# lambdaclass/mina_bridge

Hardware: AMD Instinct MI355X
Metric: Mina state proofs verified/sec (batch) (higher is better)
Workload: dtype u32x8-montgomery (255-bit prime fields, integer)

## Files before the change

include/mina_verify.h:

```cpp
#ifndef MINA_VERIFY_H
#define MINA_VERIFY_H

#include <stddef.h>
#include <stdint.h>

#ifdef __cplusplus
extern "C" {
#endif

#define MINA_OK 0
#define MINA_ERR_ARG (-1)
#define MINA_ERR_HIP (-2)
#define MINA_ERR_STATE (-3)
#define MINA_ERR_FORMAT (-4)

#define MINA_FIELD_FP 0
#define MINA_FIELD_FQ 1
#define MINA_CURVE_PALLAS 0
#define MINA_CURVE_VESTA 1

typedef struct mina_ctx mina_ctx;

int mina_ctx_create(int device_id, mina_ctx **out);
void mina_ctx_destroy(mina_ctx *ctx);
// ... 67 lines not shown

int mina_to_group(mina_ctx *ctx, int curve, size_t n, const uint8_t *t, uint8_t *out_affine);

int mina_field_mul(mina_ctx *ctx, int field, size_t n, const uint8_t *a, const uint8_t *b, uint8_t *out);
int mina_field_inv(mina_ctx *ctx, int field, size_t n, const uint8_t *a, uint8_t *out);
int mina_field_sqrt(mina_ctx *ctx, int field, size_t n, const uint8_t *a, uint8_t *out, uint8_t *out_is_square);
int mina_selftest_group_law(mina_ctx *ctx, int curve, size_t n, const uint8_t *p_affine, const uint8_t *q_affine,
                            uint8_t *out_serial, uint8_t *out_quad, uint8_t *same);
#define MINA_FE29_IN_OPERANDS 8
#define MINA_FE29_OUT_RESULTS 4
#define MINA_FE29_FLAG_NEG 1
#define MINA_FE29_FLAG_OK 1
#define MINA_FE29_FLAG_INF 2
#define MINA_FE29_MUL_ASM 0
#define MINA_FE29_SQR_ASM 1
#define MINA_FE29_DOT2_ASM 2
#define MINA_FE29_DOT3_ASM 3
#define MINA_FE29_SQR_HI_ASM 4
#define MINA_FE29_MUL_HI_ASM 5
#define MINA_FE29_MUL_LZ 6
#define MINA_FE29_SQR_LZ 7
#define MINA_FE29_MUL_HI_LZ 8
#define MINA_FE29_MULRC_LZ 9
#define MINA_FE29_DOT2RC_LZ 10
#define MINA_FE29_DOT3RC_LZ 11
#define MINA_FE29_MUL_SG 12
#define MINA_FE29_SQR_SG 13
#define MINA_FE29_MUL_HI_SG 14
#define MINA_FE29_SQR_HI_SG 15
#define MINA_FE29_MULRC_SG 16
#define MINA_FE29_DOT2RC_SG 17
#define MINA_FE29_DOT3RC_SG 18
#define MINA_FE29_ROW1_SG 19
#define MINA_FE29_SUB_KP_ONE 32
#define MINA_FE29_KP_MINUS_NEG_Y 33
#define MINA_FE29_KP_MINUS_SUB_X1 34
#define MINA_FE29_KP_MINUS_SUB_Y1 35
#define MINA_FE29_KP_MINUS_G_U1 36
#define MINA_FE29_KP_MINUS_G_S1 37
#define MINA_FE29_KP_MINUS_A_2B_X3_SUB 38
#define MINA_FE29_KP_MINUS_A_2B_G_X3_SUB 39
#define MINA_FE29_ADD_KP_MINUS_SUB_X3 40
#define MINA_FE29_ADD_KP_MINUS_G_SUB_X3 41
#define MINA_FE29_ADD 42
#define MINA_FE29_ADD3 43
#define MINA_FE29_WORDS 44
#define MINA_FE29_IS_MULTIPLE_OF_P 45
#define MINA_FE29_LEAVE 46
#define MINA_FE29_ADD_AFFINE 64
#define MINA_FE29_ADD_AFFINE_TWIN 65
#define MINA_FE29_XYZZ_ADD 66
#define MINA_FE29_XYZZ_LEAVE 67
int mina_selftest_fe29(mina_ctx *ctx, int field, int op, size_t n, const uint32_t *rows_in , uint32_t *rows_out );
#define MINA_FE32_IN_OPERANDS 8
#define MINA_FE32_OUT_RESULTS 4
#define MINA_FE32_FLAG_TRUE 1
#define MINA_FE32_FLAG_LANES_AGREE 2
#define MINA_FE32_COND_SUB_P 0
#define MINA_FE32_ADD 1
#define MINA_FE32_SUB 2
#define MINA_FE32_NEG 3
#define MINA_FE32_DBL 4
#define MINA_FE32_MUL 5
#define MINA_FE32_SQR 6
#define MINA_FE32_DOT2 7
#define MINA_FE32_DOT3 8
// ... 350 lines not shown
```

mina_bridge_amd/csrc/api_account.hip:

```cpp
#include <mutex>

#include "ctx.h"
#include <chrono>
#include <new>
#include "sponge.cuh"
#include "wire_account.h"

int mb_merkle_fold_dev(mina_ctx *c, int field, size_t n, uint32_t depth, const uint32_t *d_leaves, const uint32_t *d_sib, const uint8_t *d_dirs, uint32_t *d_roots);
int mb_merkle_prepare_salts(mina_ctx *c, int field, uint32_t depth);
int mb_ensure_state_salts(mina_ctx *c);

namespace mb {

template <int F, int LANES>
__global__ void __launch_bounds__(256)
salted_hash_kernel(uint32_t n, FieldK fk, const PoseidonParams *__restrict__ pp, const fe_t *__restrict__ salts, const uint32_t *__restrict__ salt_idx,
                   const uint32_t *__restrict__ records , const uint32_t *__restrict__ nfields,
                   const uint32_t *__restrict__ patch_a, uint32_t slot_a, const uint32_t *__restrict__ patch_b, uint32_t slot_b, uint32_t *__restrict__ out ) {
    __builtin_amdgcn_s_setprio(3);
    bool writer;
    const uint32_t sp = coop_sponge_index<LANES>(writer), e = coop_elem<LANES>();
    const bool live = sp < n;
    const uint32_t idx = live ? sp : 0;
    const uint32_t *rec = records + (size_t)idx * MINA_PSTATE_SLOTS * 8;
    uint32_t nf = nfields[idx]; if (nf > MINA_PSTATE_SLOTS) nf = MINA_PSTATE_SLOTS;
    fe_t s = salts[salt_idx[idx] * 3 + e];
    uint32_t count = 0;
    for (uint32_t el = 0; el < nf; ++el) {
        if (count == 2) { poseidon_permute_coop<F, LANES>(s, pp); count = 0; }
        if (e == count) {
            const uint32_t *src = (patch_a && el == slot_a) ? patch_a + (size_t)idx * 8 : ((patch_b && el == slot_b) ? patch_b + (size_t)idx * 8 : rec + (size_t)el * 8);
            s = fe_add<F>(s, fe_to_mont<F>(load_fe<F>(src), fk.r2));
        }
        ++count;
    }
    poseidon_permute_coop<F, LANES>(s, pp);
    s = coop_get<LANES>(s, 0);
    if (live && writer) { const fe_t w = fe_from_mont<F>(s); for (int i = 0; i < 8; ++i) out[(size_t)sp * 8 + i] = w.v[i]; }
}

}

static int salted_hash_dev(mina_ctx *c, size_t n, const uint32_t *salt_idx, const uint32_t *recs, const uint32_t *nf, const uint32_t *pa, uint32_t sa,
                           const uint32_t *pb, uint32_t sb, uint32_t *out) {
    const PoseidonParams *pp = c->pparams[FIELD_FP].as<PoseidonParams>();
    const fe_t *salts = c->state_salts.as<fe_t>();
    ProfScope ps_(c, PS_STATE_HASH);
    return with_lanes<16, 8, 3>(hash_lanes(c, n, n), [&](auto lanes) {
        constexpr int LN = decltype(lanes)::value;
        mb::salted_hash_kernel<FIELD_FP, LN><<<cdiv(coop_threads<LN>(n), 256), 256, 0, c->L->stream>>>((uint32_t)n, c->fk[FIELD_FP], pp, salts, salt_idx, recs, nf, pa, sa, pb, sb, out);
        HIPC(hipGetLastError());
        return MINA_OK;
    });
}

namespace {
struct ParsedAccount { bool ok = false, abi_ok = false; mw::Account acc; uint32_t depth = 0; uint8_t sib[64 * 32]; uint8_t dirs[64]; uint8_t ledger[32]; };

void parse_account(const uint8_t *proof, size_t proof_len, const uint8_t *pub, size_t pub_len, ParsedAccount &pa) {
    if (!proof || !pub) return;
    size_t acc_off = 0, eo = 0, el = 0;
    if (mina_parse_merkle_path(proof, proof_len, 64, pa.sib, pa.dirs, &pa.depth, &acc_off) != MINA_OK) return;
    if (mina_parse_account_pub_inputs(pub, pub_len, pa.ledger, &eo, &el) != MINA_OK) return;
    mw::Bincode c(proof + acc_off, proof_len - acc_off);
    if (!mw::read_account(c, pa.acc) || c.pos != proof_len - acc_off) return;
    pa.ok = true;
    std::vector<uint8_t> enc;
    mw::abi_encode_account(pa.acc, enc);
    pa.abi_ok = enc.size() == el && memcmp(enc.data(), pub + eo, el) == 0;
}

}

static int account_hashes(mina_ctx *c, const std::vector<const mw::Account *> &accs, uint8_t *hashes_out, uint32_t depth, const uint8_t *sib, const uint8_t *dirs, uint8_t *roots_out,
                          Lane *lane = nullptr, std::mutex *enq_mu = nullptr) {
    const size_t n = accs.size();
    if (n == 0) return MINA_OK;
    int rc;
    struct Enq {
        mina_ctx *c; Lane *lane; std::mutex *mu; bool held = false;
        void lock() { if (mu) mu->lock(); held = true; if (lane) c->L = lane; else c->use_lane0(); }
// ... 127 lines not shown
```

mina_bridge_amd/csrc/api_account_dev.hip:

```cpp
#include <mutex>

#include "ctx.h"
#include "account_pack.cuh"
#include "wire_account.h"

int mb_merkle_prepare_salts(mina_ctx *c, int field, uint32_t depth);
int mb_ensure_state_salts(mina_ctx *c);

static_assert(mb::ACCT_SALT_URI == MB_SALT_ZKAPP_URI && mb::ACCT_SALT_VK == MB_SALT_SIDE_LOADED_VK && mb::ACCT_SALT_ZKAPP == MB_SALT_ZKAPP_ACCOUNT && mb::ACCT_SALT_ACCOUNT == MB_SALT_ACCOUNT &&
              mb::ACCT_SALT_VK == MB_N_PREFIX_SALTS - 1, "account_pack.cuh names the salts of ctx.h");
static_assert(mb::ZR_URI_HASH == mw::ZK_SLOT_URI && mb::ZR_VK_HASH == mw::ZK_SLOT_VK, "the zkApp record's patched slots (wire_account.h)");

static constexpr size_t ACCOUNT_MAX_PROOFS = (size_t)1 << 22;
static constexpr size_t REC_BYTES = (size_t)MINA_PSTATE_SLOTS * 32;

static int acct_hash_dev(mina_ctx *c, size_t n, uint32_t roles, const uint32_t *count_dev, const uint32_t *salt_idx, const uint32_t *recs, const uint32_t *nf, const uint32_t *pa, uint32_t sa,
                         const uint32_t *pb, uint32_t sb, const uint32_t *marks, const uint32_t *pa_default, const uint32_t *out_index, uint32_t *out) {
    const PoseidonParams *pp = c->pparams[FIELD_FP].as<PoseidonParams>();
    const fe_t *salts = c->state_salts.as<fe_t>();
    ProfScope ps_(c, PS_STATE_HASH);
    return with_lanes<16, 8, 3>(hash_lanes(c, n, n * roles), [&](auto lanes) {
        constexpr int LN = decltype(lanes)::value;
        mb::acct_hash_kernel<FIELD_FP, LN><<<cdiv(coop_threads<LN>(n * roles), 256), 256, 0, c->L->stream>>>((uint32_t)n, roles, count_dev, c->fk[FIELD_FP], pp, salts, salt_idx, recs, nf, pa, sa,
                                                                                                           pb, sb, marks, pa_default, out_index, out);
        HIPC(hipGetLastError());
        return MINA_OK;
    });
}

static constexpr size_t DEF_RECS = 96, DEF_NF = DEF_RECS + 3 * REC_BYTES, DEF_SALT = DEF_NF + 12, DEF_BYTES = DEF_SALT + 12;
static int ensure_defaults(mina_ctx *c) {
    if (c->have_acct_defaults) return MINA_OK;
    int rc;
    if ((rc = c->acct_defaults.ensure(DEF_BYTES))) return rc;
    std::vector<uint8_t> host(DEF_BYTES, 0);
    uint32_t *nf = (uint32_t *)(host.data() + DEF_NF), *salt = (uint32_t *)(host.data() + DEF_SALT);
    const mw::ZkappAccount z;
    std::vector<mw::B32> f;
    auto put = [&](size_t k, uint32_t salt_id) { for (size_t j = 0; j < f.size() && j < MINA_PSTATE_SLOTS; ++j) memcpy(host.data() + DEF_RECS + k * REC_BYTES + j * 32, f[j].b, 32);
                                                 nf[k] = (uint32_t)(f.size() < MINA_PSTATE_SLOTS ? f.size() : MINA_PSTATE_SLOTS); salt[k] = salt_id; };
    mw::zkapp_uri_fields(z.zkapp_uri, f); put(0, MB_SALT_ZKAPP_URI);
    mw::vk_fields(mw::dummy_vk(), f); put(1, MB_SALT_SIDE_LOADED_VK);
    mw::zkapp_fields(z, f); put(2, MB_SALT_ZKAPP_ACCOUNT);
    uint8_t *d = c->acct_defaults.as<uint8_t>();
    uint32_t *h = c->acct_defaults.as<uint32_t>();
    HIPC(hipMemcpyAsync(d, host.data(), DEF_BYTES, hipMemcpyHostToDevice, c->L->stream));
    const uint32_t *recs = (const uint32_t *)(d + DEF_RECS), *dnf = (const uint32_t *)(d + DEF_NF), *dsalt = (const uint32_t *)(d + DEF_SALT);
    if ((rc = acct_hash_dev(c, 1, 2, nullptr, dsalt, recs, dnf, nullptr, 0, nullptr, 0, nullptr, nullptr, nullptr, h))) return rc;
    if ((rc = acct_hash_dev(c, 1, 1, nullptr, dsalt + 2, recs + 2 * REC_BYTES / 4, dnf + 2, h, mw::ZK_SLOT_URI, h + 8, mw::ZK_SLOT_VK, nullptr, nullptr, nullptr, h + 16))) return rc;
    HIPC(hipStreamSynchronize(c->L->stream));
    c->have_acct_defaults = true;
    return MINA_OK;
}

// ... 18 lines not shown
    }
};

static int frontend_launch(mina_ctx *c, size_t n, const void *d_blob, size_t blob_len, const void *d_proof_off, const void *d_proof_len, const void *d_pub_off, const void *d_pub_len,
                           void *d_records, void *d_nfields, void *d_salt_idx, void *d_siblings, void *d_dirs, void *d_depths, void *d_ledger, void *d_marks, void *d_zk_index,
                           void *d_zk_count, void *d_bits) {
    HIPC(hipMemsetAsync(d_zk_count, 0, 4, c->L->stream));
    mb::acct_frontend_kernel<<<cdiv(n, 256), 256, 0, c->L->stream>>>((uint32_t)n, (const uint8_t *)d_blob, (uint64_t)blob_len, (const uint64_t *)d_proof_off, (const uint64_t *)d_proof_len,
                                                                   (const uint64_t *)d_pub_off, (const uint64_t *)d_pub_len, (uint4 *)d_records, (uint32_t *)d_nfields, (uint32_t *)d_salt_idx,
                                                                   (uint4 *)d_siblings, (uint8_t *)d_dirs, (uint32_t *)d_depths, (uint4 *)d_ledger, (uint32_t *)d_marks, (uint32_t *)d_zk_index,
                                                                   (uint32_t *)d_zk_count, (uint32_t *)d_bits);
    HIPC(hipGetLastError());
    return MINA_OK;
}

static int account_job_on_lane(mina_ctx *c, size_t n, const void *d_blob, size_t blob_len, const void *d_proof_off, const void *d_proof_len, const void *d_pub_off, const void *d_pub_len,
                               void *d_passed, void *d_ran, void *d_account_hashes, void *d_roots) {
    Lane &L = *c->L;
    const AccountWs w(n);
    int rc;
    if ((rc = L.ac_ws.ensure(w.total))) return rc;
    uint8_t *d = L.ac_ws.as<uint8_t>();
    auto W = [&](size_t off) { return (uint32_t *)(d + off); };
    auto stage = [&](size_t off, uint32_t s, size_t per) { return (const uint32_t *)(d + off + (size_t)s * n * per); };
    if ((rc = frontend_launch(c, n, d_blob, blob_len, d_proof_off, d_proof_len, d_pub_off, d_pub_len, d + w.records, d + w.nfields, d + w.salt_idx, d + w.siblings, d + w.dirs, d + w.depths,
                              d + w.ledger, d + w.marks, d + w.zk_index, d + w.zk_count, d + w.bits))) return rc;
    const uint32_t *defaults = c->acct_defaults.as<uint32_t>(), *zk_count = W(w.zk_count);
    if ((rc = acct_hash_dev(c, n, 2, zk_count, stage(w.salt_idx, mb::AS_URI, 4), stage(w.records, mb::AS_URI, REC_BYTES), stage(w.nfields, mb::AS_URI, 4), nullptr, 0, nullptr, 0, nullptr, nullptr,
                            nullptr, W(w.h_uri)))) return rc;
    if ((rc = acct_hash_dev(c, n, 1, zk_count, stage(w.salt_idx, mb::AS_ZKAPP, 4), stage(w.records, mb::AS_ZKAPP, REC_BYTES), stage(w.nfields, mb::AS_ZKAPP, 4), W(w.h_uri), mw::ZK_SLOT_URI,
                            W(w.h_uri) + n * 8, mw::ZK_SLOT_VK, nullptr, nullptr, W(w.zk_index), W(w.h_zkapp)))) return rc;
    if ((rc = acct_hash_dev(c, n, 1, nullptr, stage(w.salt_idx, mb::AS_ACCOUNT, 4), stage(w.records, mb::AS_ACCOUNT, REC_BYTES), stage(w.nfields, mb::AS_ACCOUNT, 4), W(w.h_zkapp), mb::AR_ZKAPP_HASH,
                            nullptr, 0, W(w.marks), defaults + 16, nullptr, W(w.h_account)))) return rc;
    if ((rc = with_lanes<16, 8, 3>(merkle_lanes(c, n), [&](auto lanes) {
            constexpr int LN = decltype(lanes)::value;
            mb::acct_fold_kernel<FIELD_FP, LN><<<cdiv(coop_threads<LN>(n), 256), 256, 0, L.stream>>>((uint32_t)n, c->fk[FIELD_FP], c->pparams[FIELD_FP].as<PoseidonParams>(),
                c->merkle_salts[FIELD_FP].as<fe_t>(), W(w.h_account), W(w.siblings), d + w.dirs, W(w.depths), W(w.roots));
            HIPC(hipGetLastError());
            return MINA_OK;
        }))) return rc;
    mb::acct_verdict_kernel<<<cdiv(n, 256), 256, 0, L.stream>>>((uint32_t)n, W(w.bits), (const uint4 *)(d + w.roots), (const uint4 *)(d + w.ledger), (uint32_t *)d_passed, (uint32_t *)d_ran);
    HIPC(hipGetLastError());
    if (d_account_hashes) HIPC(hipMemcpyAsync(d_account_hashes, d + w.h_account, n * 32, hipMemcpyDeviceToDevice, L.stream));
    if (d_roots) HIPC(hipMemcpyAsync(d_roots, d + w.roots, n * 32, hipMemcpyDeviceToDevice, L.stream));
    return MINA_OK;
}

static bool misaligned8(const void *a, const void *b, const void *c2, const void *d) { return (((uintptr_t)a | (uintptr_t)b | (uintptr_t)c2 | (uintptr_t)d) & 7u) != 0; }

extern "C" int mina_account_frontend_dev(mina_ctx *c, size_t n, const void *d_blob, size_t blob_len, const void *d_proof_off, const void *d_proof_len, const void *d_pub_off,
                                         const void *d_pub_len, void *d_records, void *d_nfields, void *d_salt_idx, void *d_siblings, void *d_dirs, void *d_depths, void *d_ledger_hashes,
                                         void *d_zk_marks, void *d_zk_index, void *d_zk_count, void *d_bits) {
    if (!c || !d_zk_count || (n && (!d_blob || !d_proof_off || !d_proof_len || !d_pub_off || !d_pub_len || !d_records || !d_nfields || !d_salt_idx || !d_siblings || !d_dirs || !d_depths ||
                                    !d_ledger_hashes || !d_zk_marks || !d_zk_index || !d_bits))) return fail(MINA_ERR_ARG, "null argument");
    if (misaligned8(d_proof_off, d_proof_len, d_pub_off, d_pub_len) || (((uintptr_t)d_records | (uintptr_t)d_siblings | (uintptr_t)d_ledger_hashes) & 15u) ||
        (((uintptr_t)d_nfields | (uintptr_t)d_salt_idx | (uintptr_t)d_depths | (uintptr_t)d_zk_marks | (uintptr_t)d_zk_index | (uintptr_t)d_zk_count | (uintptr_t)d_bits) & 3u))
        return fail(MINA_ERR_ARG, "misaligned argument: offsets / lengths 8, records / siblings / ledger hashes 16, the u32 arrays 4 bytes");
    if (n > ACCOUNT_MAX_PROOFS) return fail(MINA_ERR_ARG, "n too large");
    if (!c->have_pparams[FIELD_FP]) return fail(MINA_ERR_STATE, "Poseidon constants not installed for Fp");
    HIPC(hipSetDevice(c->device));
    c->next_lane();
    if (n == 0) { HIPC(hipMemsetAsync(d_zk_count, 0, 4, c->L->stream)); return MINA_OK; }
    return frontend_launch(c, n, d_blob, blob_len, d_proof_off, d_proof_len, d_pub_off, d_pub_len, d_records, d_nfields, d_salt_idx, d_siblings, d_dirs, d_depths, d_ledger_hashes, d_zk_marks,
                           d_zk_index, d_zk_count, d_bits);
}

extern "C" int mina_account_job_dev(mina_ctx *c, size_t n, const void *d_blob, size_t blob_len, const void *d_proof_off, const void *d_proof_len, const void *d_pub_off, const void *d_pub_len,
// ... 59 lines not shown
```

mina_bridge_amd/csrc/api_core.hip:

```cpp
#include "ctx.h"
#include "sponge.cuh"
#include "msm.cuh"

#include <sys/random.h>
#include <atomic>
#include <condition_variable>
#include <deque>
#include <mutex>

template <int F> static fe_t host_modulus() { fe_t p; for (int i = 0; i < 8; ++i) p.v[i] = modulus_limb<F>(i); return p; }
static void fe_shr1(fe_t &a) { for (int i = 0; i < 7; ++i) a.v[i] = (a.v[i] >> 1) | (a.v[i + 1] << 31); a.v[7] >>= 1; }
static fe_t fe_sub_small(const fe_t &a, uint32_t k) { fe_t r = a; uint64_t br = k; for (int i = 0; i < 8 && br; ++i) { uint64_t t = (uint64_t)r.v[i] - br; r.v[i] = (uint32_t)t; br = (t >> 32) & 1u; } return r; }
static fe_t fe_div3(const fe_t &a) { fe_t r; uint64_t rem = 0; for (int i = 7; i >= 0; --i) { uint64_t cur = (rem << 32) | a.v[i]; r.v[i] = (uint32_t)(cur / 3); rem = cur % 3; } return r; }

template <int F> static FieldK make_field_consts() {
    FieldK k;
    fe_t p = host_modulus<F>();
    fe_t a = fe_zero(); a.v[0] = 1;
    for (int i = 0; i < 512; ++i) { a = fe_add<F>(a, a); if (i == 255) k.one = a; }
    k.r2 = a;
    fe_t pm1 = fe_sub_small(p, 1);
    k.pm2 = fe_sub_small(p, 2);
    k.pm1d2 = pm1; fe_shr1(k.pm1d2);
    k.half = k.pm1d2;
// ... 24 lines not shown
    if (ndev <= 0) return fail(MINA_ERR_HIP, "no HIP device: libminaverify has no CPU fallback");
    if (device_id < 0 || device_id >= ndev) return fail(MINA_ERR_ARG, "bad device id");
    HIPC(hipSetDevice(device_id));
    mina_ctx *c = new mina_ctx();
    c->device = device_id;
    hipError_t e = hipStreamCreateWithFlags(&c->lanes[0].stream, hipStreamNonBlocking);
    if (e != hipSuccess) { delete c; return fail(MINA_ERR_HIP, "hipStreamCreate failed"); }
    c->use_lane0();
    c->fk[FIELD_FP] = make_field_consts<FIELD_FP>();
    c->fk[FIELD_FQ] = make_field_consts<FIELD_FQ>();
    c->state_frontend = mb_state_frontend_on_lane;
    c->account_on_device = mb_verify_account_dev_on;
    *out = c;
    return MINA_OK;
}

int mb_ctx_create_view(mina_ctx *parent, mina_ctx **out) {
    if (!parent || !out) return fail(MINA_ERR_ARG, "null argument");
    int rc = mina_ctx_create(parent->device, out);
    if (rc) return rc;
    (*out)->is_view = true;
    mb_ctx_refresh_view(*out, parent);
    return MINA_OK;
}
void mb_ctx_refresh_view(mina_ctx *v, mina_ctx *p) {
    for (int i = 0; i < 2; ++i) {
        v->fk[i] = p->fk[i];
        SrsState &a = v->srs[i]; const SrsState &b = p->srs[i];
        a.depth = b.depth; a.c = b.c; a.W = b.W;
        a.table.alias(b.table); a.table29.alias(b.table29); a.table29s.alias(b.table29s); a.h.alias(b.h);
        if (a.srs_gen != b.srs_gen || a.lagrange_log2 != b.lagrange_log2 || (a.lagrange_host.empty() && !b.lagrange_host.empty())) { a.lagrange_host = b.lagrange_host; a.lagrange_log2 = b.lagrange_log2; a.srs_gen = b.srs_gen; }
        a.lagrange_table.alias(b.lagrange_table); a.lagrange_table_n = b.lagrange_table_n; a.lagrange_table_log2 = b.lagrange_table_log2;
        a.lagrange_digits.alias(b.lagrange_digits); a.lagrange_digits29.alias(b.lagrange_digits29); a.lagrange_digits_n = b.lagrange_digits_n;
        v->pparams[i].alias(p->pparams[i]); v->have_pparams[i] = p->have_pparams[i]; v->pparams_surrogate[i] = p->pparams_surrogate[i]; v->pparams_rows1[i] = p->pparams_rows1[i];
        v->merkle_salts[i].alias(p->merkle_salts[i]); v->merkle_depth[i] = p->merkle_depth[i];
    }
    v->kimchi_index.alias(p->kimchi_index); v->kimchi_tokens.alias(p->kimchi_tokens); v->kimchi_literals.alias(p->kimchi_literals);
    v->have_kimchi = p->have_kimchi; v->kimchi_log2 = p->kimchi_log2; memcpy(v->kimchi_digest, p->kimchi_digest, sizeof v->kimchi_digest); memcpy(v->kimchi_comms_host, p->kimchi_comms_host, sizeof v->kimchi_comms_host);
    v->pickles_index.alias(p->pickles_index); v->pickles_tokens.alias(p->pickles_tokens); v->pickles_literals.alias(p->pickles_literals);
    v->have_pickles_dev = p->have_pickles_dev; v->pickles_ms_valid = p->pickles_ms_valid;
    if (v->step_host && v->step_host_free && v->step_host != p->step_host) v->step_host_free(v->step_host);
    v->step_host = p->step_host; v->step_host_free = nullptr;
    v->state_salts.alias(p->state_salts); v->have_state_salts = p->have_state_salts;
}

extern "C" void mina_ctx_destroy(mina_ctx *c) {
    if (!c) return;
    (void)hipSetDevice(c->device);
    for (int i = 0; i < MB_MAX_LANES; ++i) if (c->lanes[i].stream) (void)hipStreamSynchronize(c->lanes[i].stream);
    for (int i = 0; i < 2; ++i) { c->srs[i].table.release(); c->srs[i].table29.release(); c->srs[i].table29s.release(); c->srs[i].h.release(); c->srs[i].lagrange_table.release(); c->srs[i].lagrange_digits.release(); c->srs[i].lagrange_digits29.release(); c->pparams[i].release(); c->merkle_salts[i].release(); }
    c->state_salts.release(); c->acct_defaults.release(); c->dedup_totals.release(); c->kimchi_index.release(); c->kimchi_tokens.release(); c->kimchi_literals.release();
    c->pickles_index.release(); c->pickles_tokens.release(); c->pickles_literals.release();
    if (c->step_host && c->step_host_free) c->step_host_free(c->step_host);
    c->step_host = nullptr;
    for (int i = 0; i < MB_MAX_LANES; ++i) c->lanes[i].release_all();
    for (auto &r : c->prof.recs) { (void)hipEventDestroy(r.a); (void)hipEventDestroy(r.b); }
    for (int i = 0; i < MB_MAX_LANES; ++i) {
        Lane &L = c->lanes[i];
        if (L.aux) { (void)hipStreamSynchronize(L.aux); (void)hipStreamDestroy(L.aux); (void)hipEventDestroy(L.ev_fork); (void)hipEventDestroy(L.ev_join); }
        if (L.ev_leg) (void)hipEventDestroy(L.ev_leg);
        if (L.stream) (void)hipStreamDestroy(L.stream);
    }
    delete c;
}

__attribute__((constructor)) static void mb_default_hw_queues() { setenv("GPU_MAX_HW_QUEUES", "16", 0); }

// ... 207 lines not shown
```

mina_bridge_amd/csrc/api_ipa.hip:

```cpp
#include "ctx.h"
#include "msm.cuh"
#include "sponge.cuh"

namespace mb {

enum : uint8_t {
    TAPE_ABSORB_FQ = 0,
    TAPE_ABSORB_G = 1,
    TAPE_ABSORB_FR = 2,
    TAPE_CHALLENGE = 3,
    TAPE_CHALLENGE_FQ = 4,
    TAPE_CHALLENGE_ENDO = 5,
    TAPE_DIGEST = 6,
    TAPE_CHALLENGE_ENDO_OWN = 7,
};
template <int CURVE, int LANES>
__global__ void __launch_bounds__(64) __attribute__((amdgpu_waves_per_eu(LANES == 3 ? 4 : 1, 8)))
sponge_tape_kernel(uint32_t batch, uint32_t tape_len, uint32_t in_stride_words, uint32_t out_stride_words, FieldK kb, FieldK ks,
                   const PoseidonParams *__restrict__ pp, const uint8_t *__restrict__ tape, const uint32_t *__restrict__ init_state ,
                   const uint32_t *__restrict__ init_pos , const uint32_t *__restrict__ inputs, uint32_t *__restrict__ outputs,
                   uint32_t *__restrict__ final_state , uint32_t *__restrict__ final_pos ) {
    constexpr int FB = (CURVE == CURVE_PALLAS) ? FIELD_FP : FIELD_FQ;
    constexpr int FS = (CURVE == CURVE_PALLAS) ? FIELD_FQ : FIELD_FP;
    bool writer_; const uint32_t b = coop_sponge_index<LANES>(writer_), qq = coop_elem<LANES>();
// ... 425 lines not shown
    if ((rc = h2d(c, c->L->ipa_in_b, sg, count * 64))) return rc;
    return accumulator_check_each(c, curve, k, count, verdicts);
}

int mb_ipa_batch_check_dev(mina_ctx *c, int curve, mb::IpaShape sh, const mb::IpaDevIn &in, uint32_t *d_verdict, const FoldExport *fx) {
    SrsState &s = c->srs[curve];
    const int FB = base_field_of(curve), FS = scalar_field_of(curve);
    const size_t batch = sh.batch; const uint32_t k = sh.k;
    int rc;
    if (fx) sh.pow_first = 1;
    if (sh.nshared && (sh.ncomms > 64 || sh.nshared > 64)) return fail(MINA_ERR_ARG, "shared entries need <= 64 commitments");
    const size_t npoints = batch * sh.per + sh.nshared;
    if ((rc = c->L->ipa_points.ensure(npoints * sizeof(affine_t)))) return rc;
    if ((rc = c->L->ipa_scalars.ensure(npoints * 32))) return rc;
    if ((rc = c->L->ipa_chals.ensure(batch * k * 32))) return rc;
    if ((rc = c->L->ipa_sigma.ensure(batch * 32))) return rc;
    if ((rc = c->L->ipa_folded.ensure(((size_t)1 << k) * 32))) return rc;
    if ((rc = c->L->ipa_xyzz_a.ensure(sizeof(xyzz_t)))) return rc;
    if ((rc = c->L->ipa_xyzz_b.ensure(sizeof(xyzz_t)))) return rc;
    if (sh.nshared) { if ((rc = c->L->ipa_shared.ensure(batch * sh.nshared * 32))) return rc; if ((rc = c->L->ipa_shared_off.ensure(sh.nshared * 4))) return rc; }
    HIPC(hipMemsetAsync(d_verdict, 0, 8, c->L->stream));
    const PoseidonParams *pp = c->pparams[FB].as<PoseidonParams>();
    { ProfScope ps_(c, PS_IPA_TRANSCRIPT);
    {
        const mina_verify_tuning tune = mb_tune();
        Lane &L = *c->L;
        if ((rc = L.ipa_xfer.ensure(batch * mb::IPA_XFER_WORDS * 4))) return rc;
        const bool side = c->nlanes == 1 && tune.ipa_side_stream != 0 && !c->is_view;
        hipStream_t tg = L.stream;
        if (side) {
            if (!L.aux) { HIPC(hipStreamCreateWithFlags(&L.aux, hipStreamNonBlocking)); HIPC(hipEventCreateWithFlags(&L.ev_fork, hipEventDisableTiming)); HIPC(hipEventCreateWithFlags(&L.ev_join, hipEventDisableTiming)); }
            tg = L.aux;
        }
        const int ln = transcript_lanes(c, batch, (size_t)tune.ipa_coop8_max);
        auto prepare = [&](auto phase) {
            return with_lanes<16, 8, 3>(ln, [&](auto lanes) {
                constexpr int LN = decltype(lanes)::value, PH = decltype(phase)::value;
                DISPATCH_CURVE(curve, {
                    mb::ipa_prepare_kernel<C_, LN, PH><<<cdiv(coop_threads<LN>(batch), 64), 64, 0, L.stream>>>(
                        sh, c->fk[FB], c->fk[FS], pp, in.state, in.pos, in.cip, in.lr, in.delta, in.sg, in.z1, in.z2, in.pts, in.r,
                        in.xi, in.comms, in.comm_override, in.expand, in.rb, in.sb, s.h.as<affine_t>(), L.ipa_points.as<affine_t>(), L.ipa_scalars.as<uint32_t>(),
                        L.ipa_chals.as<uint32_t>(), L.ipa_sigma.as<uint32_t>(), d_verdict + 1, L.ipa_xfer.as<uint32_t>(), L.ipa_shared.as<uint32_t>(), L.ipa_shared_off.as<uint32_t>());
                });
                return MINA_OK;
            });
        };
        if ((rc = prepare(std::integral_constant<int, 1>{}))) return rc;
        if (side) { HIPC(hipEventRecord(L.ev_fork, L.stream)); HIPC(hipStreamWaitEvent(L.aux, L.ev_fork, 0)); }
        DISPATCH_FIELD(FB, { mb::ipa_to_group_kernel<F_><<<cdiv(batch, 64), 64, 0, tg>>>((uint32_t)batch, sh.per, c->fk[F_], L.ipa_xfer.as<uint32_t>(), L.ipa_points.as<affine_t>()); });
        if (side) HIPC(hipEventRecord(L.ev_join, L.aux));
        if ((rc = prepare(std::integral_constant<int, 2>{}))) return rc;
        if (side) HIPC(hipStreamWaitEvent(L.stream, L.ev_join, 0));
    }
    }
    HIPC(hipGetLastError());
    if (sh.nshared) { DISPATCH_FIELD(FS, { mb::ipa_shared_tail_kernel<F_><<<sh.nshared, 256, 0, c->L->stream>>>(sh.batch, sh.nshared, sh.per, c->L->ipa_shared.as<uint32_t>(), c->L->ipa_scalars.as<uint32_t>()); }); }
    if ((rc = mb_bpoly_fold(c, FS, k, batch, c->L->ipa_chals.as<uint32_t>(), c->L->ipa_sigma.as<uint32_t>(), c->L->ipa_folded.as<uint32_t>()))) return rc;
    if (fx) {
        HIPC(hipMemcpyAsync(fx->ipa_scalars, c->L->ipa_folded.p, ((size_t)1 << k) * 32, hipMemcpyDeviceToDevice, c->L->stream));
        if ((rc = mb_msm_variable(c, curve, (uint32_t)npoints, c->L->ipa_scalars.as<uint32_t>(), c->L->ipa_points.p, fx->ipa_point, nullptr))) return rc;
        fold_export_flag_kernel<<<1, 64, 0, c->L->stream>>>(d_verdict + 1, d_verdict);
        HIPC(hipGetLastError());
        return MINA_OK;
    }
    if ((rc = mb_msm_fixed(c, curve, 1u << k, c->L->ipa_folded.as<uint32_t>(), nullptr, c->L->ipa_xyzz_a.p))) return rc;
    if ((rc = mb_msm_variable(c, curve, (uint32_t)npoints, c->L->ipa_scalars.as<uint32_t>(), c->L->ipa_points.p, nullptr, c->L->ipa_xyzz_b.p))) return rc;
    DISPATCH_FIELD(FB, { xyzz_compare_kernel<F_><<<1, 64, 0, c->L->stream>>>(c->L->ipa_xyzz_a.as<xyzz_t>(), c->L->ipa_xyzz_b.as<xyzz_t>(), 1, d_verdict, d_verdict + 1); });
// ... 87 lines not shown

extern "C" int mina_fq_sponge_run(mina_ctx *c, int curve, size_t batch, const uint8_t *tape, size_t tape_len, const uint8_t *init_state,
                                  const uint32_t *init_pos, const uint8_t *inputs, uint8_t *outputs, uint8_t *final_state, uint32_t *final_pos) {
    if (!c || !tape || (batch && tape_len && !outputs && !final_state)) return fail(MINA_ERR_ARG, "null argument");
    if (curve != 0 && curve != 1) return fail(MINA_ERR_ARG, "bad curve");
    if ((init_state == nullptr) != (init_pos == nullptr)) return fail(MINA_ERR_ARG, "init_state and init_pos go together");
    if (batch == 0) return MINA_OK;
    if (batch > (1u << 22) || tape_len > (1u << 16)) return fail(MINA_ERR_ARG, "batch or tape too large");
    const int FB = base_field_of(curve);
    if (!c->have_pparams[FB]) return fail(MINA_ERR_STATE, "Poseidon constants not installed for the base field");
    size_t in_words = 0, out_words = 0;
    for (size_t t = 0; t < tape_len; ++t) {
        switch (tape[t]) {
            case TAPE_ABSORB_FQ: case TAPE_ABSORB_FR: in_words += 8; break;
            case TAPE_ABSORB_G: in_words += 16; break;
            case TAPE_CHALLENGE: case TAPE_CHALLENGE_FQ: case TAPE_CHALLENGE_ENDO: case TAPE_DIGEST: case TAPE_CHALLENGE_ENDO_OWN: out_words += 8; break;
            default: return fail(MINA_ERR_ARG, "unknown tape opcode");
        }
    }
    if ((in_words && !inputs) || (out_words && !outputs)) return fail(MINA_ERR_ARG, "null argument");
    if (init_pos) for (size_t b = 0; b < batch; ++b) if (init_pos[2 * b] > 1 || init_pos[2 * b + 1] > 2) return fail(MINA_ERR_ARG, "bad sponge position");
    HIPC(hipSetDevice(c->device));
    c->use_lane0();
    int rc;
    Lane &L = *c->L;
    if ((rc = h2d(c, L.ipa_in_a, tape, tape_len))) return rc;
    if ((rc = h2d(c, L.ipa_in_b, inputs, batch * in_words * 4))) return rc;
    if (init_state) { if ((rc = h2d(c, L.ipa_in_c, init_state, batch * 96))) return rc; if ((rc = h2d(c, L.ipa_sigma, init_pos, batch * 8))) return rc; }
    if ((rc = L.ipa_scalars.ensure(batch * (out_words ? out_words : 8) * 4))) return rc;
    if ((rc = L.ipa_points.ensure(batch * 96))) return rc;
    if ((rc = L.ipa_chals.ensure(batch * 8))) return rc;
    const PoseidonParams *pp = c->pparams[FB].as<PoseidonParams>();
    const int FS = scalar_field_of(curve);
    if ((rc = with_lanes<8, 3>(sponge_batch_lanes(batch), [&](auto lanes) {
            constexpr int LN = decltype(lanes)::value;
            DISPATCH_CURVE(curve, {
                mb::sponge_tape_kernel<C_, LN><<<cdiv(coop_threads<LN>(batch), 64), 64, 0, L.stream>>>((uint32_t)batch, (uint32_t)tape_len, (uint32_t)in_words, (uint32_t)out_words,
                    c->fk[FB], c->fk[FS], pp, L.ipa_in_a.as<uint8_t>(), init_state ? L.ipa_in_c.as<uint32_t>() : nullptr, init_state ? L.ipa_sigma.as<uint32_t>() : nullptr,
                    L.ipa_in_b.as<uint32_t>(), L.ipa_scalars.as<uint32_t>(), L.ipa_points.as<uint32_t>(), L.ipa_chals.as<uint32_t>());
            });
            return MINA_OK;
        }))) return rc;
    HIPC(hipGetLastError());
    if (final_state) HIPC(hipMemcpyAsync(final_state, L.ipa_points.p, batch * 96, hipMemcpyDeviceToHost, L.stream));
    if (final_pos) HIPC(hipMemcpyAsync(final_pos, L.ipa_chals.p, batch * 8, hipMemcpyDeviceToHost, L.stream));
    return d2h_sync(c, outputs, L.ipa_scalars, batch * out_words * 4);
}
```

mina_bridge_amd/csrc/api_kimchi.hip:

```cpp
#include "ctx.h"
#include "msm.cuh"
#include "sponge.cuh"
#include "wire_proof.h"
#include "kimchi_dev.cuh"

namespace mb {

struct KimchiIndexDev {
    uint32_t log2_domain, zk_rows, perm_alpha_offset, n_tokens;
    fe_t shifts[7];
    fe_t omega, omega_zk, n_inv, zk_roots[KC_MAX_ZK];
    fe_t mds[9], endo_coeff;
    fe_t digest;
    affine_t sigma6;
    uint32_t col_comm_words[(6 + 15 + 6) * 16];
};
struct KimchiIn { const uint32_t *pub, *prev_chals, *prev_comms, *w_comm, *z_comm, *t_comm, *evals, *ft_eval1, *pubcomm; };
struct KimchiOut { uint32_t *sponge_state, *sponge_pos, *cip, *evalpoints, *polyscale, *evalscale, *comms, *ft_eval0; };

__device__ __forceinline__ xyzz_t xyzz_shfl_xor(const xyzz_t &a, int mask) {
    xyzz_t r;
    for (int i = 0; i < 8; ++i) { r.x.v[i] = (uint32_t)__shfl_xor((int)a.x.v[i], mask, 64); r.y.v[i] = (uint32_t)__shfl_xor((int)a.y.v[i], mask, 64);
                                  r.zz.v[i] = (uint32_t)__shfl_xor((int)a.zz.v[i], mask, 64); r.zzz.v[i] = (uint32_t)__shfl_xor((int)a.zzz.v[i], mask, 64); }
    return r;
// ... 271 lines not shown
    int rc;
    if ((rc = c->kimchi_index.ensure(sizeof *ix))) return rc;
    if ((rc = c->kimchi_tokens.ensure((toks.size() ? toks.size() : 1) * sizeof(mb::KimchiToken)))) return rc;
    if ((rc = c->kimchi_literals.ensure(lm.size() * sizeof(fe_t)))) return rc;
    HIPC(hipMemcpy(c->kimchi_index.p, ix, sizeof *ix, hipMemcpyHostToDevice));
    if (!toks.empty()) HIPC(hipMemcpy(c->kimchi_tokens.p, toks.data(), toks.size() * sizeof(mb::KimchiToken), hipMemcpyHostToDevice));
    HIPC(hipMemcpy(c->kimchi_literals.p, lm.data(), lm.size() * sizeof(fe_t), hipMemcpyHostToDevice));
    memcpy(c->kimchi_comms_host, vi->sigma_comm, 7 * 64); memcpy(c->kimchi_comms_host + 7 * 64, vi->coefficients_comm, 15 * 64); memcpy(c->kimchi_comms_host + 22 * 64, vi->selector_comm, 6 * 64);
    c->kimchi_log2 = vi->log2_domain; c->have_kimchi = true; c->pickles_ms_valid = false;
    return MINA_OK;
}

extern "C" int mina_verifier_index_digest(mina_ctx *c, uint8_t *out32) {
    if (!c || !out32) return fail(MINA_ERR_ARG, "null argument");
    if (!c->have_kimchi) return fail(MINA_ERR_STATE, "no verifier index installed");
    memcpy(out32, c->kimchi_digest, 32);
    return MINA_OK;
}

int mb_kimchi_to_batch_dev(mina_ctx *c, size_t batch, uint32_t n_prev, uint32_t npub, const mb::KimchiIn &in, const mb::KimchiOut &out, uint32_t *d_bad, mb::IpaExpand *expand,
                           const void *pf_digest, uint32_t pf_stride) {
    if (!c->have_kimchi) return fail(MINA_ERR_STATE, "no verifier index installed");
    const PoseidonParams *ppb = c->pparams[FIELD_FP].as<PoseidonParams>(), *pps = c->pparams[FIELD_FQ].as<PoseidonParams>();
    ProfScope ps_(c, PS_KIMCHI);
    Lane &L = *c->L;
    int rc;
    if ((rc = L.kc_xfer.ensure(batch * mb::KC_XF * sizeof(fe_t)))) return rc;
    fe_t *xf = L.kc_xfer.as<fe_t>();
    const mb::KimchiIndexDev *ix = c->kimchi_index.as<mb::KimchiIndexDev>();
    const uint32_t B = (uint32_t)batch, ncomms = n_prev + 2 + mb::KC_COLS;
    const FieldK &kb = c->fk[FIELD_FP], &ks = c->fk[FIELD_FQ];
    mb::kimchi_rows_kernel<<<cdiv(batch * ncomms * 16, 256), 256, 0, L.stream>>>(B, n_prev, ix, in, out.comms);
    const uint32_t fq_roles = pf_digest ? 1u : 2u;
    if ((rc = with_lanes<16, 8, 3>(transcript_lanes(c, batch, (size_t)mb_tune().kimchi_coop8_max), [&](auto lanes) {
            constexpr int LN = decltype(lanes)::value;
            mb::kimchi_fq_kernel<LN><<<fq_roles * coop_role_blocks<LN>(batch), 64, 0, L.stream>>>(B, n_prev, kb, ks, ppb, pps, ix, in, out, xf, d_bad, coop_role_blocks<LN>(batch), (const fe_t *)pf_digest, pf_stride);
            if (npub > 32 && npub <= 40) mb::kimchi_pub_kernel<10><<<cdiv(batch * 8, 64), 64, 0, L.stream>>>(B, npub, ks, ix, in, xf, d_bad);
            else mb::kimchi_pub_kernel<8><<<cdiv(batch * 8, 64), 64, 0, L.stream>>>(B, npub, ks, ix, in, xf, d_bad);
            mb::kimchi_fr_kernel<LN><<<cdiv(coop_threads<LN>(batch), 64), 64, 0, L.stream>>>(B, ks, pps, in, xf, d_bad);
            return MINA_OK;
        }))) return rc;
    mb::kimchi_scalar_kernel<<<cdiv(batch, 64), 64, 0, L.stream>>>(B, n_prev, ks, ix, c->kimchi_tokens.as<mb::KimchiToken>(), c->kimchi_literals.as<fe_t>(), in, out, xf, d_bad);
    if (expand) { expand->p0 = &ix->sigma6; expand->pts = in.t_comm; expand->sc = xf + mb::XF_FTSC; expand->stride = mb::KC_XF; }
    else mb::kimchi_ftcomm_kernel<<<cdiv(batch * 8, 64), 64, 0, L.stream>>>(B, n_prev, kb, ix, in, out, xf);
    HIPC(hipGetLastError());
    return MINA_OK;
}

int mb_ensure_lagrange_table(mina_ctx *c, int curve, uint32_t log2_domain, uint32_t npub);
int mb_pubcomm_dev(mina_ctx *c, size_t batch, uint32_t log2_domain, uint32_t npub, const uint32_t *d_pub, uint32_t *d_out16);

static int check_kimchi_in(mina_ctx *c, const mina_kimchi_proofs *p) {
    if (!c || !p) return fail(MINA_ERR_ARG, "null argument");
    if (!c->have_kimchi) return fail(MINA_ERR_STATE, "no verifier index installed");
    if (p->batch == 0 || p->batch > 65536 || p->n_prev > 8 || p->npub > 4096 || p->npub > (1u << c->kimchi_log2)) return fail(MINA_ERR_ARG, "bad batch / n_prev / npub");
    if ((p->npub && !p->public_inputs) || (p->n_prev && (!p->prev_chals || !p->prev_comms)) || !p->w_comm || !p->z_comm || !p->t_comm || !p->evals || !p->ft_eval1) return fail(MINA_ERR_ARG, "null section");
    return MINA_OK;
}

extern "C" int mina_kimchi_to_batch(mina_ctx *c, const mina_kimchi_proofs *p, mina_kimchi_batch_out *o) {
    int rc = check_kimchi_in(c, p);
    if (rc) return rc;
    if (!o || !o->sponge_state || !o->sponge_pos || !o->cip || !o->evalpoints || !o->polyscale || !o->evalscale || !o->comms) return fail(MINA_ERR_ARG, "null output");
    HIPC(hipSetDevice(c->device));
    c->use_lane0();
    const size_t B = p->batch, k = c->kimchi_log2, ncomms = p->n_prev + 2 + mb::KC_COLS;
    if (p->npub && (rc = mb_ensure_lagrange_table(c, CURVE_PALLAS, (uint32_t)k, p->npub))) return rc;
// ... 31 lines not shown
```

mina_bridge_amd/csrc/api_pickles.hip:

```cpp
#include <mutex>

#include "ctx.h"
#include "sponge.cuh"
#include "kimchi_dev.cuh"
#include "wire_proof.h"

namespace {

constexpr uint32_t SRS_LENGTH_LOG2 = 16, PERM_ALPHA0 = 21, N_STEP_COLS = 43 + 19;

template <int F> fe_t to_mont_bytes(const uint8_t *b, const FieldK &k) { fe_t a; memcpy(a.v, b, 32); return fe_to_mont<F>(a, k.r2); }
template <int F> fe_t from_u128(const mw::Chal128 &c, const FieldK &k) {
    fe_t a = fe_zero(); a.v[0] = (uint32_t)c.lo; a.v[1] = (uint32_t)(c.lo >> 32); a.v[2] = (uint32_t)c.hi; a.v[3] = (uint32_t)(c.hi >> 32); return fe_to_mont<F>(a, k.r2);
}
template <int F> void put_plain(std::vector<uint8_t> &v, const fe_t &mont) { const fe_t p = fe_from_mont<F>(mont); const uint8_t *b = (const uint8_t *)p.v; v.insert(v.end(), b, b + 32); }
template <int F> fe_t bpoly_host(const std::vector<fe_t> &chals, fe_t x, const FieldK &k) {
    fe_t acc = k.one;
    for (size_t i = chals.size(); i-- > 0;) { acc = fe_mul<F>(acc, fe_add<F>(k.one, fe_mul<F>(chals[i], x))); x = fe_sqr<F>(x); }
    return acc;
}
template <int F> fe_t reduce_256(const uint8_t *b, const FieldK &k) {
    fe_t lo = fe_zero(), hi = fe_zero();
    memcpy(lo.v, b, 16); memcpy(hi.v, b + 16, 16);
    fe_t two128 = fe_zero(); two128.v[4] = 1;
// ... 408 lines not shown
    if (!ok) ok_out[b] = 0u;
}

}

int mb_pickles_dev(mina_ctx *c, size_t batch, const mb::PicklesIn &in, uint32_t *d_pub, uint32_t *d_ok) {
    if (!c->have_pickles_dev) return fail(MINA_ERR_STATE, "no step index installed");
    if (!c->have_kimchi) return fail(MINA_ERR_STATE, "no wrap verifier index installed");
    if (in.n_old > 4 || in.n_evals < mb::KC_COLS || in.n_evals > N_STEP_COLS) return fail(MINA_ERR_ARG, "bad n_old / n_evals");
    Lane &L = *c->L;
    int rc;
    if (!c->pickles_ms_valid) {
        Lane *keep = c->L;
        std::vector<uint8_t> tape(28, MINA_TAPE_ABSORB_G), stt(96); uint32_t pos[2];
        std::vector<uint8_t> dummy(32);
        if ((rc = mina_fq_sponge_run(c, CURVE_PALLAS, 1, tape.data(), tape.size(), nullptr, nullptr, c->kimchi_comms_host, dummy.data(), stt.data(), pos))) return rc;
        HIPC(hipStreamSynchronize(c->L->stream));
        mb::PicklesIndexDev *ixd = c->pickles_index.as<mb::PicklesIndexDev>();
        fe_t ms[3]; for (int e = 0; e < 3; ++e) ms[e] = to_mont_bytes<FIELD_FP>(stt.data() + 32 * e, c->fk[FIELD_FP]);
        HIPC(hipMemcpy(&ixd->ms_state, ms, sizeof ms, hipMemcpyHostToDevice));
        HIPC(hipMemcpy(&ixd->ms_squeezed, pos, 8, hipMemcpyHostToDevice));
        c->pickles_ms_valid = true;
        c->L = keep;
    }
    const mb::PicklesIndexDev *ix = c->pickles_index.as<mb::PicklesIndexDev>();
    if ((rc = L.pk_xe.ensure(batch * mb::px_stride(in.n_old) * sizeof(fe_t)))) return rc;
    fe_t *xe = L.pk_xe.as<fe_t>();
    const FieldK &kp = c->fk[FIELD_FP], &kq = c->fk[FIELD_FQ];
    const PoseidonParams *ppp = c->pparams[FIELD_FP].as<PoseidonParams>(), *ppq = c->pparams[FIELD_FQ].as<PoseidonParams>();
    const uint32_t B = (uint32_t)batch;
    ProfScope ps_(c, PS_PICKLES);
    HIPC(hipMemsetD32Async((hipDeviceptr_t)d_ok, 1, batch, L.stream));
    mb::pickles_expand_kernel<<<cdiv(batch * (50 + 16 * in.n_old), 256), 256, 0, L.stream>>>(B, kp, kq, in, xe);
    if ((rc = with_lanes<16, 8, 3>(transcript_lanes(c, batch, 1024), [&](auto lanes) {
            constexpr int LN = decltype(lanes)::value;
            mb::pickles_digest_kernel<LN><<<3 * coop_role_blocks<LN>(batch), 64, 0, L.stream>>>(B, kp, kq, ppp, ppq, ix, in, xe, d_ok, coop_role_blocks<LN>(batch));
            mb::pickles_tick_kernel<LN><<<cdiv(coop_threads<LN>(batch), 64), 64, 0, L.stream>>>(B, kp, ppp, in, xe, d_ok);
            return MINA_OK;
        }))) return rc;
    mb::pickles_scalar_kernel<<<cdiv(batch, 64), 64, 0, L.stream>>>(B, kp, kq, ix, c->pickles_tokens.as<mb::KimchiToken>(), c->pickles_literals.as<fe_t>(), in, xe, d_pub, d_ok);
    HIPC(hipGetLastError());
    return MINA_OK;
}

static mb::PicklesIn pickles_in_of(const mina_pickles_statements &s) {
    auto W = [](const void *p) { return (const uint32_t *)p; };
    return mb::PicklesIn{s.n_old, s.n_evals, W(s.plonk), W(s.bulletproof_challenges), W(s.step_old_challenges), W(s.step_comms), W(s.wrap_old_challenges), W(s.wrap_sg),
                         W(s.sponge_digest), W(s.prev_evals), W(s.prev_public_input), W(s.prev_ft_eval1), W(s.app_state), (const uint8_t *)s.misc};
}
int mb_pickles_check(mina_ctx *c, const mina_pickles_statements *s) {
    if (!s || !s->plonk || !s->bulletproof_challenges || (s->n_old && (!s->step_old_challenges || !s->step_comms)) || !s->wrap_old_challenges || !s->wrap_sg || !s->sponge_digest ||
        !s->prev_evals || !s->prev_public_input || !s->prev_ft_eval1 || !s->app_state || !s->misc) return fail(MINA_ERR_ARG, "null statement section");
    if (s->n_old > 4 || s->n_evals < mb::KC_COLS || s->n_evals > N_STEP_COLS) return fail(MINA_ERR_ARG, "bad n_old / n_evals");
    if (!c->have_pickles_dev) return fail(MINA_ERR_STATE, "no step index installed");
    if (!c->have_kimchi) return fail(MINA_ERR_STATE, "no wrap verifier index installed");
    return MINA_OK;
}
int mb_pickles_statements_dev(mina_ctx *c, size_t batch, const mina_pickles_statements *s, uint32_t *d_pub, uint32_t *d_ok) { return mb_pickles_dev(c, batch, pickles_in_of(*s), d_pub, d_ok); }
void mb_pickles_kimchi_digest(mina_ctx *c, const mina_pickles_statements *s, const void **first, uint32_t *stride) {
    *first = c->L->pk_xe.as<fe_t>() + mb::px_kdig(s->n_old); *stride = mb::px_stride(s->n_old);
}
size_t mb_pickles_sections(const mina_pickles_statements *s, const void ***slots , size_t *strides , mina_pickles_statements *copy) {
    *copy = *s;
    const void **sl[12] = {&copy->plonk, &copy->bulletproof_challenges, &copy->step_old_challenges, &copy->step_comms, &copy->wrap_old_challenges, &copy->wrap_sg, &copy->sponge_digest,
                           &copy->prev_evals, &copy->prev_public_input, &copy->prev_ft_eval1, &copy->app_state, &copy->misc};
    const size_t st[12] = {64, 256, (size_t)s->n_old * 256, (size_t)s->n_old * 64, 480, 64, 32, (size_t)s->n_evals * 64, 64, 32, 32, 32};
    for (int i = 0; i < 12; ++i) { slots[i] = sl[i]; strides[i] = st[i]; }
// ... 55 lines not shown
```

mina_bridge_amd/csrc/api_selftest.hip:

```cpp
#include "ctx.h"
#include "ec29.cuh"
#include "groupmap.cuh"

static constexpr uint32_t FE29_IN_WORDS = MINA_FE29_IN_OPERANDS * 9 + 1, FE29_OUT_WORDS = MINA_FE29_OUT_RESULTS * 9 + 1;

#define FE29_OPS(X)                                                                                                                                                  \
    X(MINA_FE29_MUL_ASM) X(MINA_FE29_SQR_ASM) X(MINA_FE29_DOT2_ASM) X(MINA_FE29_DOT3_ASM) X(MINA_FE29_SQR_HI_ASM) X(MINA_FE29_MUL_HI_ASM)                            \
    X(MINA_FE29_MUL_LZ) X(MINA_FE29_SQR_LZ) X(MINA_FE29_MUL_HI_LZ) X(MINA_FE29_MULRC_LZ) X(MINA_FE29_DOT2RC_LZ) X(MINA_FE29_DOT3RC_LZ)                               \
    X(MINA_FE29_MUL_SG) X(MINA_FE29_SQR_SG) X(MINA_FE29_MUL_HI_SG) X(MINA_FE29_SQR_HI_SG) X(MINA_FE29_MULRC_SG) X(MINA_FE29_DOT2RC_SG) X(MINA_FE29_DOT3RC_SG)        \
    X(MINA_FE29_ROW1_SG)                                                                                                                                             \
    X(MINA_FE29_SUB_KP_ONE) X(MINA_FE29_KP_MINUS_NEG_Y) X(MINA_FE29_KP_MINUS_SUB_X1) X(MINA_FE29_KP_MINUS_SUB_Y1) X(MINA_FE29_KP_MINUS_G_U1) X(MINA_FE29_KP_MINUS_G_S1) \
    X(MINA_FE29_KP_MINUS_A_2B_X3_SUB) X(MINA_FE29_KP_MINUS_A_2B_G_X3_SUB) X(MINA_FE29_ADD_KP_MINUS_SUB_X3) X(MINA_FE29_ADD_KP_MINUS_G_SUB_X3)                        \
    X(MINA_FE29_ADD) X(MINA_FE29_ADD3) X(MINA_FE29_WORDS) X(MINA_FE29_IS_MULTIPLE_OF_P) X(MINA_FE29_LEAVE)                                                           \
    X(MINA_FE29_ADD_AFFINE) X(MINA_FE29_ADD_AFFINE_TWIN) X(MINA_FE29_XYZZ_ADD) X(MINA_FE29_XYZZ_LEAVE)

template <int F, int OP>
__global__ void __launch_bounds__(64)
fe29_selftest_kernel(uint32_t n, fe_t one, fe_t m32, const uint32_t *__restrict__ in, uint32_t *__restrict__ out) {
#if defined(__HIP_DEVICE_COMPILE__)
    const uint32_t row = OP == MINA_FE29_ROW1_SG ? blockIdx.x : blockIdx.x * blockDim.x + threadIdx.x;
    if (row >= n) return;
    const uint32_t *w = in + (size_t)row * FE29_IN_WORDS;
    fe29_t s[MINA_FE29_IN_OPERANDS], o[MINA_FE29_OUT_RESULTS];
#pragma unroll
    for (int k = 0; k < MINA_FE29_IN_OPERANDS; ++k)
#pragma unroll
        for (int i = 0; i < L29; ++i) s[k].v[i] = w[k * L29 + i];
    const uint32_t flag = w[FE29_IN_WORDS - 1];
#pragma unroll
    for (int k = 0; k < MINA_FE29_OUT_RESULTS; ++k) o[k] = fe29_zero();
    uint32_t oflag = 0;
    auto words_out = [&](int k, const fe_t &x) {
#pragma unroll
        for (int i = 0; i < 8; ++i) o[k].v[i] = x.v[i];
    };
    if constexpr (OP == MINA_FE29_MUL_ASM) o[0] = fe29_mul_asm<F>(s[0], s[1]);
    else if constexpr (OP == MINA_FE29_SQR_ASM) o[0] = fe29_sqr_asm<F>(s[0]);
    else if constexpr (OP == MINA_FE29_DOT2_ASM) o[0] = fe29_dot2_asm<F>(s[0], s[1], s[2], s[3]);
    else if constexpr (OP == MINA_FE29_DOT3_ASM) o[0] = fe29_dot3_asm<F>(s[0], s[1], s[2], s[3], s[4], s[5]);
    else if constexpr (OP == MINA_FE29_SQR_HI_ASM) o[0] = fe29_sqr_hi_asm<F>(s[0], s[7]);
    else if constexpr (OP == MINA_FE29_MUL_HI_ASM) o[0] = fe29_mul_hi_asm<F>(s[0], s[1], s[7]);
    else if constexpr (OP == MINA_FE29_MUL_LZ) o[0] = fe29_mul_lz<F>(s[0], s[1]);
    else if constexpr (OP == MINA_FE29_SQR_LZ) o[0] = fe29_sqr_lz<F>(s[0]);
    else if constexpr (OP == MINA_FE29_MUL_HI_LZ) o[0] = fe29_mul_hi_lz<F>(s[0], s[1], s[7]);
    else if constexpr (OP == MINA_FE29_MULRC_LZ) o[0] = fe29_mulrc_lz<F>(s[0], s[1], s[6]);
    else if constexpr (OP == MINA_FE29_DOT2RC_LZ) o[0] = fe29_dot2rc_lz<F>(s[0], s[1], s[2], s[3], s[6]);
    else if constexpr (OP == MINA_FE29_DOT3RC_LZ) o[0] = fe29_dot3rc_lz<F>(s[0], s[1], s[2], s[3], s[4], s[5], s[6]);
    else if constexpr (OP == MINA_FE29_MUL_SG) o[0] = fe29_mul_sg<F>(s[0], s[1]);
    else if constexpr (OP == MINA_FE29_SQR_SG) o[0] = fe29_sqr_sg<F>(s[0]);
    else if constexpr (OP == MINA_FE29_MUL_HI_SG) o[0] = fe29_mul_hi_sg<F>(s[0], s[1], s[7]);
    else if constexpr (OP == MINA_FE29_SQR_HI_SG) o[0] = fe29_sqr_hi_sg<F>(s[0], s[7]);
    else if constexpr (OP == MINA_FE29_MULRC_SG) o[0] = fe29_mulrc_sg<F>(s[0], s[1], s[6]);
    else if constexpr (OP == MINA_FE29_DOT2RC_SG) o[0] = fe29_dot2rc_sg<F>(s[0], s[1], s[2], s[3], s[6]);
    else if constexpr (OP == MINA_FE29_DOT3RC_SG) o[0] = fe29_dot3rc_sg<F>(s[0], s[1], s[2], s[3], s[4], s[5], s[6]);
    else if constexpr (OP == MINA_FE29_ROW1_SG) o[0] = fe29_row1_sg<F>(s[7], s[0], s[1], s[2], s[3], s[6]);
    else if constexpr (OP == MINA_FE29_SUB_KP_ONE) o[0] = fe29_sub_kp<F, 1>(s[0], s[1]);
    else if constexpr (OP == MINA_FE29_KP_MINUS_NEG_Y) o[0] = fe29_kp_minus<F, EC29::NEG_Y_MULT>(s[0]);
    else if constexpr (OP == MINA_FE29_KP_MINUS_SUB_X1) o[0] = fe29_kp_minus<F, EC29::SUB_X1_MULT>(s[0]);
    else if constexpr (OP == MINA_FE29_KP_MINUS_SUB_Y1) o[0] = fe29_kp_minus<F, EC29::SUB_Y1_MULT>(s[0]);
    else if constexpr (OP == MINA_FE29_KP_MINUS_G_U1) o[0] = fe29_kp_minus<F, EC29::G_U1_MULT>(s[0]);
    else if constexpr (OP == MINA_FE29_KP_MINUS_G_S1) o[0] = fe29_kp_minus<F, EC29::G_S1_MULT>(s[0]);
    else if constexpr (OP == MINA_FE29_KP_MINUS_A_2B_X3_SUB) o[0] = fe29_kp_minus_a_minus_2b<F, EC29::X3_SUB_MULT>(s[0], s[1]);
    else if constexpr (OP == MINA_FE29_KP_MINUS_A_2B_G_X3_SUB) o[0] = fe29_kp_minus_a_minus_2b<F, EC29::G_X3_SUB_MULT>(s[0], s[1]);
    else if constexpr (OP == MINA_FE29_ADD_KP_MINUS_SUB_X3) o[0] = fe29_add_kp_minus<F, EC29::SUB_X3_MULT>(s[0], s[1]);
    else if constexpr (OP == MINA_FE29_ADD_KP_MINUS_G_SUB_X3) o[0] = fe29_add_kp_minus<F, EC29::G_SUB_X3_MULT>(s[0], s[1]);
    else if constexpr (OP == MINA_FE29_ADD) o[0] = fe29_add(s[0], s[1]);
    else if constexpr (OP == MINA_FE29_ADD3) o[0] = fe29_add3(s[0], s[1], s[2]);
    else if constexpr (OP == MINA_FE29_WORDS) {
        fe_t x;
#pragma unroll
        for (int i = 0; i < 8; ++i) x.v[i] = s[0].v[i];
        o[0] = fe29_from_words(x); words_out(1, fe29_to_words(o[0]));
    }
    else if constexpr (OP == MINA_FE29_IS_MULTIPLE_OF_P) oflag = fe29_is_multiple_of_p<F>(s[0]) ? 1u : 0u;
    else if constexpr (OP == MINA_FE29_LEAVE) words_out(0, fe29_leave<F>(s[0], fe29_from_words(one)));
    else {
        xyzz29_t acc; acc.x = s[0]; acc.y = s[1]; acc.zz = s[2]; acc.zzz = s[3];
        bool inf = (flag & MINA_FE29_FLAG_INF) != 0, ok = true;
        if constexpr (OP == MINA_FE29_ADD_AFFINE) { inf = false; ok = xyzz29_add_affine<F>(acc, inf, s[4], s[5], [&]() { return s[5]; }, []() {}, m32); }
        else if constexpr (OP == MINA_FE29_ADD_AFFINE_TWIN) ok = xyzz29_add_affine<F>(acc, inf, s[4], s[5], (flag & MINA_FE29_FLAG_NEG) != 0, m32);
        else if constexpr (OP == MINA_FE29_XYZZ_ADD) { xyzz29_t b; b.x = s[4]; b.y = s[5]; b.zz = s[6]; b.zzz = s[7]; inf = false; ok = xyzz29_add<F>(acc, b); }
        else static_assert(OP == MINA_FE29_XYZZ_LEAVE, "unknown op");
        if constexpr (OP == MINA_FE29_XYZZ_LEAVE) {
            const xyzz_t v = xyzz29_leave<F>(acc, inf, one);
            words_out(0, v.x); words_out(1, v.y); words_out(2, v.zz); words_out(3, v.zzz);
        } else { o[0] = acc.x; o[1] = acc.y; o[2] = acc.zz; o[3] = acc.zzz; }
        oflag = (ok ? MINA_FE29_FLAG_OK : 0u) | (inf ? MINA_FE29_FLAG_INF : 0u);
    }
// ... 148 lines not shown
```

mina_bridge_amd/csrc/api_sponge.hip:

```cpp
#include "ctx.h"
#include "sponge.cuh"
#include "bpoly_mfma.cuh"

static BpolyShape bp_shape(uint32_t k, size_t batch) { BpolyShape s; s.k = k; s.lb = k / 2; s.hb = k - s.lb; s.batch = (uint32_t)batch; return s; }

template <int F>
static int run_bpoly_fold(mina_ctx *c, uint32_t k, size_t batch, const uint32_t *d_chals, const uint32_t *d_weights, uint32_t *d_out) {
    BpolyShape sh = bp_shape(k, batch);
    const uint32_t nl = 1u << sh.lb, nh = 1u << sh.hb, n = 1u << k;
    const uint32_t lo_blocks = cdiv(nl, 256), hi_tiles = cdiv(nh, BP_HT);
    uint32_t slices = 1;
    while (slices * 2 <= batch && (size_t)lo_blocks * hi_tiles * slices < 2048 && slices < 64) slices *= 2;
    int rc;
    if (batch == 1 && !d_weights) {
        ProfScope ps_(c, PS_BPOLY_FOLD);
        bpoly_single_kernel<F><<<cdiv(nl, 256) * cdiv(nh, BP1_HT), nl < 256 ? (nl < 64 ? 64 : nl) : 256, 0, c->L->stream>>>(sh, c->fk[F], d_chals, nullptr, d_out);
        HIPC(hipGetLastError());
        return MINA_OK;
    }
    const bool mfma_on = mb_tune().bpoly_mfma != 0;
    if (mfma_on && batch >= 256 && batch < (1u << 17) && sh.lb >= 1) {
        Lane &L = *c->L;
        const uint32_t kpad = (uint32_t)(cdiv(batch, BPM_KALIGN) * BPM_KALIGN);
        if ((rc = L.bp_ldig.ensure((size_t)nl * BPM_DIGITS * kpad)) || (rc = L.bp_hdig.ensure((size_t)nh * BPM_DIGITS * kpad)) ||
// ... 81 lines not shown
    auto load = [&](size_t idx) { fe_t w; memcpy(w.v, params + idx * 32, 32); return fe_to_mont<F>(w, fk.r2); };
    for (int i = 0; i < 3; ++i) for (int j = 0; j < 3; ++j) pp.mds[i][j] = load(3 * i + j);
    for (int r = 0; r < 55; ++r) for (int j = 0; j < 3; ++j) pp.rc[r][j] = load(9 + 3 * r + j);
}

template <int F> static bool poseidon_rows1(const PoseidonParams &pp, const FieldK &k, const fe_t &two5, const fe_t &two522, PoseidonRows1 &out) {
    for (int i = 0; i < 3; ++i) if (fe_is_zero(pp.mds[i][i])) return false;
    auto pow7 = [&](const fe_t &a) { const fe_t a2 = fe_mul<F>(a, a), a4 = fe_mul<F>(a2, a2); return fe_mul<F>(fe_mul<F>(a4, a2), a); };
    auto to29 = [&](const fe_t &a, const fe_t &scale) { return fe29_from_words(fe_mul<F>(a, scale)); };
    fe_t minv[3], d[3] = {k.one, k.one, k.one};
    for (int i = 0; i < 3; ++i) minv[i] = fe_inv<F>(pp.mds[i][i], k);
    for (int r = 0; r < 55; ++r) {
        fe_t d7inv[3], dn[3];
        for (int j = 0; j < 3; ++j) { const fe_t d7 = pow7(d[j]); d7inv[j] = fe_inv<F>(d7, k); dn[j] = r < 54 ? fe_mul<F>(d7, minv[j]) : k.one; }
        for (int i = 0; i < 3; ++i) {
            fe_t a[3];
            for (int j = 0; j < 3; ++j) a[j] = fe_mul<F>(fe_mul<F>(dn[i], pp.mds[i][j]), d7inv[j]);
            const fe_t rc = fe_mul<F>(dn[i], pp.rc[r][i]);
            if (r < 54) {
                if (!fe_eq(a[i], k.one)) return false;
                PoseidonRow1 &w = out.row[r][i];
                w.a[0] = to29(a[i == 2 ? 0 : i + 1], two5); w.a[1] = to29(a[i == 0 ? 2 : i - 1], two5); w.rc = to29(rc, two522);
            } else {
                for (int j = 0; j < 3; ++j) out.last[i][j] = to29(a[j], two5);
                out.last_rc[i] = to29(rc, two522);
            }
        }
        for (int j = 0; j < 3; ++j) d[j] = dn[j];
    }
    out.ok = 1;
    return true;
}

bool mb_params_are_surrogate(int field, const uint8_t *params);
extern "C" int mina_poseidon_set_params(mina_ctx *c, int field, const uint8_t *params) {
    if (!c || !params) return fail(MINA_ERR_ARG, "null argument");
    if (bad_field(field)) return fail(MINA_ERR_ARG, "bad field");
    HIPC(hipSetDevice(c->device));
    c->use_lane0();
    struct { PoseidonParams pp; PoseidonParams29 q; PoseidonRows1 q1; } both;
    PoseidonParams &pp = both.pp;
    static_assert(sizeof(both) == sizeof(PoseidonParams) + sizeof(PoseidonParams29) + sizeof(PoseidonRows1), "PoseidonParams29 sits right behind PoseidonParams, PoseidonRows1 behind it");
    memset(&both, 0, sizeof both);
    DISPATCH_FIELD(field, {
        params_to_mont<F_>(params, c->fk[F_], pp);
        const FieldK &k = c->fk[F_];
        fe_t two5 = fe_zero(); two5.v[0] = 1u << 5; two5 = fe_to_mont<F_>(two5, k.r2);
        for (int i = 0; i < 3; ++i) for (int j = 0; j < 3; ++j) both.q.mds[i][j] = fe29_from_words(fe_mul<F_>(pp.mds[i][j], two5));
        for (int r = 0; r < 55; ++r) for (int i = 0; i < 3; ++i) both.q.rc[r][i] = fe29_from_words(fe_mul<F_>(pp.rc[r][i], two5));
        both.q.enter = fe29_from_words(fe_mul<F_>(two5, two5));
        const fe_t two522 = fe_to_mont<F_>(fe_mul<F_>(two5, two5), k.r2);
        for (int r = 0; r < 55; ++r) for (int i = 0; i < 3; ++i) both.q.rc2[r][i] = fe29_from_words(fe_mul<F_>(pp.rc[r][i], two522));
        both.q.absorb = fe29_from_words(two522);
        both.q.leave = fe29_from_words(k.one);
        if (!poseidon_rows1<F_>(pp, k, two5, two522, both.q1)) memset(&both.q1, 0, sizeof both.q1);
    });
    int rc;
    if ((rc = c->pparams[field].ensure(sizeof both))) return rc;
    HIPC(hipMemcpyAsync(c->pparams[field].p, &both, sizeof both, hipMemcpyHostToDevice, c->L->stream));
    HIPC(hipStreamSynchronize(c->L->stream));
    c->have_pparams[field] = true;
    c->pparams_rows1[field] = both.q1.ok != 0;
    c->pparams_surrogate[field] = mb_params_are_surrogate(field, params);
    c->merkle_depth[field] = 0;
    if (field == FIELD_FP) { c->have_state_salts = false; c->have_acct_defaults = false; }
    return MINA_OK;
}

static int poseidon_permute_on_lane(mina_ctx *c, int field, size_t n, void *d_states);
extern "C" int mina_poseidon_permute_dev(mina_ctx *c, int field, size_t n, void *d_states) {
    if (!c || !d_states) return fail(MINA_ERR_ARG, "null argument");
    HIPC(hipSetDevice(c->device));
    c->next_lane();
    return poseidon_permute_on_lane(c, field, n, d_states);
}
static int poseidon_permute_on_lane(mina_ctx *c, int field, size_t n, void *d_states) {
    if (bad_field(field)) return fail(MINA_ERR_ARG, "bad field");
    if (!c->have_pparams[field]) return fail(MINA_ERR_STATE, "Poseidon constants not installed for this field");
    if (n == 0) return MINA_OK;
    HIPC(hipSetDevice(c->device));
    DISPATCH_FIELD(field, { poseidon_permute_kernel<F_><<<cdiv(n, 256), 256, 0, c->L->stream>>>((uint32_t)n, c->fk[F_], c->pparams[field].as<PoseidonParams>(), (uint32_t *)d_states); });
    HIPC(hipGetLastError());
    return MINA_OK;
}

extern "C" int mina_poseidon_permute(mina_ctx *c, int field, size_t n, uint8_t *states) {
    if (!c || (n && !states)) return fail(MINA_ERR_ARG, "null argument");
    if (n == 0) return MINA_OK;
    int rc;
    HIPC(hipSetDevice(c->device));
    c->use_lane0();
    if ((rc = h2d(c, c->L->tmp_a, states, n * 96))) return rc;
    if ((rc = poseidon_permute_on_lane(c, field, n, c->L->tmp_a.p))) return rc;
    return d2h_sync(c, states, c->L->tmp_a, n * 96);
}

extern "C" int mina_poseidon_hash(mina_ctx *c, int field, size_t n, size_t len, const uint8_t *inputs, uint8_t *out) {
    if (!c || (n && !out) || (n && len && !inputs)) return fail(MINA_ERR_ARG, "null argument");
    if (bad_field(field)) return fail(MINA_ERR_ARG, "bad field");
    if (!c->have_pparams[field]) return fail(MINA_ERR_STATE, "Poseidon constants not installed for this field");
    if (n == 0) return MINA_OK;
    HIPC(hipSetDevice(c->device));
    c->use_lane0();
    int rc;
    if ((rc = h2d(c, c->L->tmp_a, inputs, n * len * 32))) return rc;
    if ((rc = c->L->tmp_c.ensure(n * 32))) return rc;
    if ((rc = with_lanes<8, 3>(sponge_batch_lanes(n), [&](auto lanes) {
            constexpr int LN = decltype(lanes)::value;
            DISPATCH_FIELD(field, { poseidon_hash_coop_kernel<F_, LN><<<cdiv(coop_threads<LN>(n), 256), 256, 0, c->L->stream>>>((uint32_t)n, (uint32_t)len, c->fk[F_], c->pparams[field].as<PoseidonParams>(), c->L->tmp_a.as<uint32_t>(), c->L->tmp_c.as<uint32_t>()); });
            return MINA_OK;
        }))) return rc;
    return d2h_sync(c, out, c->L->tmp_c, n * 32);
}

extern "C" int mina_challenge_to_field(mina_ctx *c, int field, size_t n, const uint8_t *chal128, uint8_t *out) {
    if (!c || (n && (!chal128 || !out))) return fail(MINA_ERR_ARG, "null argument");
    if (bad_field(field)) return fail(MINA_ERR_ARG, "bad field");
    if (n == 0) return MINA_OK;
    HIPC(hipSetDevice(c->device));
    c->use_lane0();
    int rc;
    if ((rc = h2d(c, c->L->tmp_a, chal128, n * 16))) return rc;
    if ((rc = c->L->tmp_c.ensure(n * 32))) return rc;
    DISPATCH_FIELD(field, { challenge_to_field_kernel<F_><<<cdiv(n, 64), 64, 0, c->L->stream>>>((uint32_t)n, c->fk[F_], c->L->tmp_a.as<uint32_t>(), c->L->tmp_c.as<uint32_t>()); });
    return d2h_sync(c, out, c->L->tmp_c, n * 32);
}

static int merkle_prepare_salts(mina_ctx *c, int field, uint32_t depth) {
    if (c->merkle_depth[field] >= depth) return MINA_OK;
    std::vector<uint8_t> pre((size_t)depth * 32, 0);
    for (uint32_t h = 0; h < depth; ++h) {
        char buf[32]; snprintf(buf, sizeof buf, "MinaMklTree%03u", h);
        size_t len = strlen(buf);
        for (size_t i = 0; i < 20; ++i) pre[(size_t)h * 32 + i] = (uint8_t)(i < len ? buf[i] : '*');
    }
    int rc;
    if ((rc = c->merkle_salts[field].ensure((size_t)depth * 3 * sizeof(fe_t)))) return rc;
    if ((rc = h2d(c, c->L->tmp_d, pre.data(), pre.size()))) return rc;
    DISPATCH_FIELD(field, { merkle_salt_kernel<F_><<<cdiv(depth, 64), 64, 0, c->L->stream>>>(depth, c->fk[F_], c->pparams[field].as<PoseidonParams>(), c->L->tmp_d.as<uint32_t>(), c->merkle_salts[field].as<fe_t>()); });
    HIPC(hipGetLastError());
    HIPC(hipStreamSynchronize(c->L->stream));
    c->merkle_depth[field] = depth;
    return MINA_OK;
}

int mb_merkle_fold_dev(mina_ctx *c, int field, size_t n, uint32_t depth, const uint32_t *d_leaves, const uint32_t *d_sib, const uint8_t *d_dirs, uint32_t *d_roots) {
    return with_lanes<16, 8, 3>(merkle_lanes(c, n), [&](auto lanes) {
        constexpr int LN = decltype(lanes)::value;
        DISPATCH_FIELD(field, {
            merkle_fold_coop_kernel<F_, LN><<<cdiv(coop_threads<LN>(n), 256), 256, 0, c->L->stream>>>((uint32_t)n, depth, c->fk[F_], c->pparams[field].as<PoseidonParams>(),
                c->merkle_salts[field].as<fe_t>(), d_leaves, d_sib, d_dirs, d_roots);
        });
        HIPC(hipGetLastError());
        return MINA_OK;
    });
}
int mb_merkle_prepare_salts(mina_ctx *c, int field, uint32_t depth) { return merkle_prepare_salts(c, field, depth); }

extern "C" int mina_merkle_roots(mina_ctx *c, int field, size_t n, uint32_t depth, const uint8_t *leaves, const uint8_t *siblings,
                                 const uint8_t *dirs, uint8_t *roots_out) {
    if (!c || (n && (!leaves || !roots_out)) || (n && depth && (!siblings || !dirs))) return fail(MINA_ERR_ARG, "null argument");
    if (bad_field(field)) return fail(MINA_ERR_ARG, "bad field");
    if (depth > 64) return fail(MINA_ERR_ARG, "depth must be <= 64");
    if (n > (1u << 24)) return fail(MINA_ERR_ARG, "n too large");
    if (!c->have_pparams[field]) return fail(MINA_ERR_STATE, "Poseidon constants not installed for this field");
    if (n == 0) return MINA_OK;
    HIPC(hipSetDevice(c->device));
    c->use_lane0();
    int rc;
    if (depth && (rc = merkle_prepare_salts(c, field, depth))) return rc;
    if ((rc = h2d(c, c->L->tmp_a, leaves, n * 32))) return rc;
    if ((rc = h2d(c, c->L->tmp_b, siblings, n * depth * 32))) return rc;
    if ((rc = h2d(c, c->L->tmp_d, dirs, n * depth))) return rc;
    if ((rc = c->L->tmp_c.ensure(n * 32))) return rc;
    if ((rc = mb_merkle_fold_dev(c, field, n, depth, c->L->tmp_a.as<uint32_t>(), c->L->tmp_b.as<uint32_t>(), c->L->tmp_d.as<uint8_t>(), c->L->tmp_c.as<uint32_t>()))) return rc;
    return d2h_sync(c, roots_out, c->L->tmp_c, n * 32);
}

extern "C" int mina_merkle_verify_batch(mina_ctx *c, int field, size_t n, uint32_t depth, const uint8_t *leaves, const uint8_t *siblings,
                                        const uint8_t *dirs, const uint8_t *expected_roots, uint8_t *verdicts) {
// ... 8 lines not shown
```

mina_bridge_amd/csrc/ctx.h:

```cpp
#pragma once
#include <hip/hip_runtime.h>

#include <cstdio>
#include <cstdlib>
#include <cstring>
#include <array>
#include <functional>
#include <memory>
#include <mutex>
#include <thread>
#include <algorithm>
#include <string>
#include <type_traits>
#include <utility>
#include <vector>

#include "../../include/mina_verify.h"
#include "groupmap.cuh"

using namespace mb;

struct mina_ctx;
int mb_ctx_create_view(mina_ctx *parent, mina_ctx **out);
void mb_ctx_refresh_view(mina_ctx *view, mina_ctx *parent);
// ... 88 lines not shown
                         &ipa_sigma, &ipa_in_a, &ipa_in_b, &ipa_in_c, &ipa_verdict, &ipa_xfer, &ipa_shared, &ipa_shared_off, &acc_rho_scaled,
                         &st_ok, &st_hashes, &st_pub_xyzz, &st_pubcomm, &st_flags, &st_in, &st_verdicts,
                         &dd_rep, &dd_uniq, &dd_table, &dd_counts, &pk_off, &pk_len, &pk_status, &pk_info, &pk_fmt, &ac_ws, &ac_in,
                         &kc_state, &kc_pos, &kc_cip, &kc_pts, &kc_v, &kc_u, &kc_comms, &kc_xfer, &kc_pch, &pk_xe, &pk_pub, &pk_ok};
        for (DevBuf *b : all) b->release();
        host_stage.release();
    }
};
static constexpr int MB_PIPE_LANES = 32;
static constexpr int MB_DEV_FORK_MAX = 8;
static constexpr int MB_DEV_HELPER0 = MB_PIPE_LANES + 3 * 16;
static constexpr int MB_MAX_LANES = MB_DEV_HELPER0 + 3 * MB_DEV_FORK_MAX;
enum : int { MB_SALT_PSTATE_BODY = 0, MB_SALT_PSTATE, MB_SALT_ACCOUNT, MB_SALT_ZKAPP_ACCOUNT, MB_SALT_ZKAPP_URI, MB_SALT_SIDE_LOADED_VK, MB_N_PREFIX_SALTS };

struct mina_ctx {
    int device = 0;
    ProfState prof;
    Lane lanes[MB_MAX_LANES];
    int nlanes = 1;
    unsigned rr = 0;
    int pinned = -1;
    Lane *L = nullptr;
    Lane *ipa_rows = nullptr; uint32_t ipa_rows_batch = 0, ipa_rows_k = 0, ipa_rows_per = 0, ipa_rows_nshared = 0; int ipa_rows_curve = -1;
    FieldK fk[2];
    SrsState srs[2];
    DevBuf pparams[2]; bool have_pparams[2] = {false, false};
    DevBuf merkle_salts[2]; uint32_t merkle_depth[2] = {0, 0};
    DevBuf kimchi_index, kimchi_tokens, kimchi_literals; bool have_kimchi = false; uint32_t kimchi_log2 = 0; uint8_t kimchi_digest[32] = {0};
    uint8_t kimchi_comms_host[28 * 64] = {0};
    DevBuf pickles_index, pickles_tokens, pickles_literals; bool have_pickles_dev = false, pickles_ms_valid = false;
    void *step_host = nullptr; void (*step_host_free)(void *) = nullptr;
    bool pparams_surrogate[2] = {false, false};
    bool pparams_rows1[2] = {false, false};
    DevBuf state_salts; bool have_state_salts = false;
    bool is_view = false;
    bool state_dedup = false;
    DevBuf dedup_totals; uint64_t dedup_states = 0;
    int (*state_frontend)(mina_ctx *c, size_t batch, const void *d_blob, size_t blob_len, const void *d_begin, const void *d_end, const void *d_expected_hashes,
                          const void *d_ledger_hashes, const void *d_and, void *d_records, void *d_nfields, void *d_precheck, void *d_masks) = nullptr;
    DevBuf acct_defaults; bool have_acct_defaults = false;
    int (*account_on_device)(mina_ctx *c, size_t n, const uint8_t *const *proofs, const size_t *proof_lens, const uint8_t *const *pubs, const size_t *pub_lens,
                             uint32_t *passed, uint32_t *ran, Lane *lane, std::mutex *enq_mu) = nullptr;
    uint32_t dev_fork_made = 0;
    void use_lane0() { L = &lanes[0]; }
    void next_lane() { L = pinned >= 0 ? &lanes[pinned] : &lanes[rr++ % (unsigned)nlanes]; }
};

static inline int mb_ctx_state_dedup(mina_ctx *c, bool on) {
    if (on && !c->state_dedup) {
        for (int i = 0; i < c->nlanes; ++i) if (c->lanes[i].stream && hipStreamSynchronize(c->lanes[i].stream) != hipSuccess) return MINA_ERR_HIP;
        int rc = c->dedup_totals.ensure(16);
        if (rc) return rc;
        if (hipMemsetAsync(c->dedup_totals.p, 0, 16, c->lanes[0].stream) != hipSuccess || hipStreamSynchronize(c->lanes[0].stream) != hipSuccess) return MINA_ERR_HIP;
        c->dedup_states = 0;
    }
    c->state_dedup = on;
    return MINA_OK;
}

static constexpr size_t COOP8_MAX_GROUPS = 8192;
static inline bool use_coop8(const mina_ctx *c, size_t groups) {
    const mina_verify_tuning t = mb_tune();
    return groups * (size_t)((c && !t.coop8_per_call) ? c->nlanes : 1) <= (size_t)t.coop8_max;
}

static inline bool use_coop16(const mina_ctx *c, size_t proofs) {
    return proofs * (size_t)(c ? c->nlanes : 1) <= (size_t)mb_tune().coop16_max;
}

static inline bool use_coop8_transcripts(const mina_ctx *c, size_t batch, size_t per_call_limit) {
    const size_t lim = (size_t)mb_tune().transcript_coop8_max;
    const size_t in_flight = batch * (size_t)(c ? c->nlanes : 1);
    return lim ? in_flight <= lim : ((batch <= per_call_limit && in_flight <= 2048) || in_flight <= 2560);
}

static constexpr size_t HASH1_MIN_STATES = 65536;
static inline int hash_jobs_in_flight(const mina_ctx *c) { return c->pinned >= 0 ? 1 : c->nlanes; }
static inline bool hash_one_lane(const mina_ctx *c, size_t leg_states) {
    const int jobs = hash_jobs_in_flight(c);
    return c->pparams_rows1[FIELD_FP] && jobs >= 2 && leg_states * (size_t)jobs >= HASH1_MIN_STATES;
}
static inline size_t hash_piece_states(const mina_ctx *c, size_t leg_states, uint32_t piece_waves) { return (size_t)piece_waves * (hash_one_lane(c, leg_states) ? 64u : 21u); }

static inline int hash_lanes(const mina_ctx *c, size_t proofs, size_t sponges) { return use_coop16(c, proofs) ? 16 : (use_coop8(c, sponges) ? 8 : 3); }
static inline int pstate_hash_lanes(const mina_ctx *c, size_t n, size_t leg_states) {
    return hash_one_lane(c, leg_states) ? 1 : hash_lanes(c, (n + MINA_STATES_PER_PROOF - 1) / MINA_STATES_PER_PROOF, n);
}
static inline int transcript_lanes(const mina_ctx *c, size_t batch, size_t per_call_limit) {
    return use_coop16(c, batch) ? 16 : (use_coop8_transcripts(c, batch, per_call_limit) ? 8 : 3);
}
static inline int sponge_batch_lanes(size_t n) { return n <= COOP8_MAX_GROUPS ? 8 : 3; }
static inline int merkle_lanes(const mina_ctx *c, size_t paths) { return use_coop16(c, paths) ? 16 : sponge_batch_lanes(paths); }

enum : uint32_t { MB_JOB_LEGS = 1, MB_JOB_FINISH = 2, MB_JOB_ALL = 3 };
struct StateJobCarry { uint32_t *ipa_v = nullptr, *acc_v = nullptr, *kimchi_bad = nullptr; const uint32_t *stmt_ok = nullptr; };
struct HashLaunch { uint32_t piece_waves = 0, lds_bytes = 0; };
struct FoldExport { uint32_t *ipa_scalars = nullptr, *ipa_point = nullptr, *acc_scalars = nullptr, *acc_point = nullptr; };
struct StateJobPlan {
    Lane *wrap = nullptr, *acc = nullptr, *states = nullptr;
    uint32_t phase = MB_JOB_ALL; StateJobCarry *carry = nullptr;
    uint32_t *d_stmt_out = nullptr;
    size_t hashed_early = 0;
    HashLaunch hash;
    bool acc_first = false;
    const FoldExport *fold_export = nullptr;
};
int mb_state_jobs_on_lane(mina_ctx *c, const mina_state_jobs *j, uint32_t *d_verdicts, uint32_t *d_flags, const StateJobPlan &plan = {});
int mb_verify_account_on(mina_ctx *c, size_t n, const uint8_t *const *proofs, const size_t *proof_lens, const uint8_t *const *pubs, const size_t *pub_lens,
                         uint32_t *passed, uint32_t *ran, Lane *lane, std::mutex *enq_mu);
int mb_state_frontend_on_lane(mina_ctx *c, size_t batch, const void *d_blob, size_t blob_len, const void *d_begin, const void *d_end, const void *d_expected_hashes,
                              const void *d_ledger_hashes, const void *d_and, void *d_records, void *d_nfields, void *d_precheck, void *d_masks);
int mb_verify_account_dev_on(mina_ctx *c, size_t n, const uint8_t *const *proofs, const size_t *proof_lens, const uint8_t *const *pubs, const size_t *pub_lens,
                             uint32_t *passed, uint32_t *ran, Lane *lane, std::mutex *enq_mu);
int mb_state_hashes_early(mina_ctx *c, Lane *LS, size_t ns_total, size_t lo, size_t cnt, const uint32_t *d_records, const uint32_t *d_nfields, hipEvent_t after, HashLaunch hash);

struct MbPoolJob;
std::shared_ptr<MbPoolJob> mb_pool_submit(size_t n, std::function<void(size_t)> fn);
void mb_pool_wait(const std::shared_ptr<MbPoolJob> &job);
size_t mb_pool_threads();
template <class Fn> static inline void mb_parallel_for(size_t n, Fn fn) {
    if (n < 128 || mb_pool_threads() <= 1) { for (size_t i = 0; i < n; ++i) fn(i); return; }
    mb_pool_wait(mb_pool_submit(n, std::function<void(size_t)>(fn)));
}
bool mb_secure_random(void *buf, size_t n);

// ... 68 lines not shown
```

mina_bridge_amd/csrc/fp29.cuh:

```cuda
#pragma once
#include "fp.cuh"

namespace mb {

static constexpr int L29 = 9;
struct fe29_t { uint32_t v[L29]; };
static constexpr uint32_t M29 = 0x1FFFFFFFu;

MB_HD constexpr uint32_t limb29_of(const uint32_t w0, const uint32_t w1, const uint32_t w2, const uint32_t w3, const uint32_t w4, const uint32_t w5, const uint32_t w6,
                                   const uint32_t w7, int i) {
    const uint32_t w[9] = {w0, w1, w2, w3, w4, w5, w6, w7, 0u};
    const int bit = 29 * i, q = bit >> 5, r = bit & 31;
    if (q >= 8) return 0u;
    const uint64_t two = (uint64_t)w[q] | ((uint64_t)w[q + 1] << 32);
    return (uint32_t)(two >> r) & M29;
}
template <int F> struct P29 {
#define MB_P29(i) limb29_of(1u, FieldP<F>::P1, FieldP<F>::P2, FieldP<F>::P3, 0, 0, 0, P7, i)
    static constexpr uint32_t L1 = MB_P29(1), L2 = MB_P29(2), L3 = MB_P29(3), L4 = MB_P29(4), L8 = MB_P29(8);
    static_assert(MB_P29(0) == 1u && MB_P29(8) == (1u << 22) && MB_P29(5) == 0u && MB_P29(6) == 0u && MB_P29(7) == 0u, "Pasta prime shape");
#undef MB_P29
};

MB_HD fe29_t fe29_from_words(const fe_t &a) {
// ... 17 lines not shown
#pragma unroll
    for (int i = 0; i < L29; ++i) { const uint32_t t = a.v[i] + b.v[i] + c; if (i < L29 - 1) { r.v[i] = t & M29; c = t >> 29; } else r.v[i] = t; }
    return r;
}

MB_HD fe29_t fe29_add3(const fe29_t &a, const fe29_t &b, const fe29_t &c) {
    fe29_t r; uint32_t k = 0;
#pragma unroll
    for (int i = 0; i < L29; ++i) { const uint32_t t = a.v[i] + b.v[i] + c.v[i] + k; if (i < L29 - 1) { r.v[i] = t & M29; k = t >> 29; } else r.v[i] = t; }
    return r;
}

struct EC29 {
    static constexpr uint32_t INV_X = 10;
    static constexpr uint32_t INV_Y = 2;
    static constexpr uint32_t INV_ZZ = 3;
    static constexpr uint32_t INV_ZZZ = 3;
    static constexpr uint32_t NEG_Y_MULT = 2;
    static constexpr uint32_t SUB_X1_MULT = 11;
    static constexpr uint32_t SUB_Y1_MULT = 3;
    static constexpr uint32_t X3_SUB_MULT = 7;
    static constexpr uint32_t SUB_X3_MULT = 11;
    static constexpr uint32_t PD_MAX = 14;
    static constexpr uint32_t G_U1_MULT = 3;
    static constexpr uint32_t G_S1_MULT = 3;
    static constexpr uint32_t G_X3_SUB_MULT = 7;
    static constexpr uint32_t G_SUB_X3_MULT = 10;
};
struct SPONGE29 {
    static constexpr uint32_t LANES3_STATE_MILLI_P = 4100;
    static constexpr uint32_t LANES8_STATE_MILLI_P = 4100;
    static constexpr uint32_t LANES16_STATE_MILLI_P = 6100;
    static constexpr uint32_t LANES1_STATE_MILLI_P = 6300;
};

#if defined(__HIP_DEVICE_COMPILE__)
template <int F> __device__ __forceinline__ fe29_t fe29_mul_asm(const fe29_t &a, const fe29_t &b) {
    uint64_t col, cc; fe29_t r;
    uint32_t m0, m1, m2, m3, m4, m5, m6, m7, m8;
    const uint32_t p1 = P29<F>::L1, p2 = P29<F>::L2, p3 = P29<F>::L3, p4 = P29<F>::L4, p8 = P29<F>::L8;
    asm("v_mad_u64_u32 %0, %1, %2, %3, 0"
        : "=&v"(col), "=&s"(cc) : "v"(a.v[0]), "v"(b.v[0]));
    m0 = (0u - (uint32_t)col) & M29;
    asm("v_mad_u64_u32 %0, %1, %2, 1, %0"
        : "+&v"(col), "=&s"(cc) : "v"(m0));
    col >>= 29;
    asm("v_mad_u64_u32 %0, %1, %2, %3, %0\n\tv_mad_u64_u32 %0, %1, %4, %5, %0\n\tv_mad_u64_u32 %0, %1, %6, %7, %0"
        : "+&v"(col), "=&s"(cc) : "v"(a.v[0]), "v"(b.v[1]), "v"(a.v[1]), "v"(b.v[0]), "v"(m0), "v"(p1));
    m1 = (0u - (uint32_t)col) & M29;
    asm("v_mad_u64_u32 %0, %1, %2, 1, %0"
        : "+&v"(col), "=&s"(cc) : "v"(m1));
    col >>= 29;
    asm("v_mad_u64_u32 %0, %1, %2, %3, %0\n\tv_mad_u64_u32 %0, %1, %4, %5, %0\n\tv_mad_u64_u32 %0, %1, %6, %7, %0\n\tv_mad_u64_u32 %0, %1, %8, %9, %0\n\tv_mad_u64_u32 %0, %1, %10, %11, %0"
        : "+&v"(col), "=&s"(cc) : "v"(a.v[0]), "v"(b.v[2]), "v"(a.v[1]), "v"(b.v[1]), "v"(a.v[2]), "v"(b.v[0]), "v"(m1), "v"(p1), "v"(m0), "v"(p2));
    m2 = (0u - (uint32_t)col) & M29;
    asm("v_mad_u64_u32 %0, %1, %2, 1, %0"
        : "+&v"(col), "=&s"(cc) : "v"(m2));
    col >>= 29;
    asm("v_mad_u64_u32 %0, %1, %2, %3, %0\n\tv_mad_u64_u32 %0, %1, %4, %5, %0\n\tv_mad_u64_u32 %0, %1, %6, %7, %0\n\tv_mad_u64_u32 %0, %1, %8, %9, %0\n\tv_mad_u64_u32 %0, %1, %10, %11, %0\n\tv_mad_u64_u32 %0, %1, %12, %13, %0\n\tv_mad_u64_u32 %0, %1, %14, %15, %0"
        : "+&v"(col), "=&s"(cc) : "v"(a.v[0]), "v"(b.v[3]), "v"(a.v[1]), "v"(b.v[2]), "v"(a.v[2]), "v"(b.v[1]), "v"(a.v[3]), "v"(b.v[0]), "v"(m2), "v"(p1), "v"(m1), "v"(p2), "v"(m0), "v"(p3));
    m3 = (0u - (uint32_t)col) & M29;
    asm("v_mad_u64_u32 %0, %1, %2, 1, %0"
        : "+&v"(col), "=&s"(cc) : "v"(m3));
    col >>= 29;
    asm("v_mad_u64_u32 %0, %1, %2, %3, %0\n\tv_mad_u64_u32 %0, %1, %4, %5, %0\n\tv_mad_u64_u32 %0, %1, %6, %7, %0\n\tv_mad_u64_u32 %0, %1, %8, %9, %0\n\tv_mad_u64_u32 %0, %1, %10, %11, %0\n\tv_mad_u64_u32 %0, %1, %12, %13, %0\n\tv_mad_u64_u32 %0, %1, %14, %15, %0\n\tv_mad_u64_u32 %0, %1, %16, %17, %0\n\tv_mad_u64_u32 %0, %1, %18, %19, %0"
        : "+&v"(col), "=&s"(cc) : "v"(a.v[0]), "v"(b.v[4]), "v"(a.v[1]), "v"(b.v[3]), "v"(a.v[2]), "v"(b.v[2]), "v"(a.v[3]), "v"(b.v[1]), "v"(a.v[4]), "v"(b.v[0]), "v"(m3), "v"(p1), "v"(m2), "v"(p2), "v"(m1), "v"(p3), "v"(m0), "v"(p4));
// ... 1682 lines not shown
        : "=&v"(nc), "=&s"(cc) : "v"(m8), "v"(col), "v"(b0.v[8]), "s"(a0.v[1]), "v"(b0.v[7]), "s"(a0.v[2]), "v"(b0.v[6]), "s"(a0.v[3]), "v"(b0.v[5]), "s"(a0.v[4]), "v"(b0.v[4]), "s"(a0.v[5]), "v"(b0.v[3]), "s"(a0.v[6]), "v"(b0.v[2]), "s"(a0.v[7]), "v"(b0.v[1]), "s"(a0.v[8]), "v"(b1.v[8]), "s"(a1.v[1]), "v"(b1.v[7]), "s"(a1.v[2]), "v"(b1.v[6]), "s"(a1.v[3]), "v"(b1.v[5]), "s"(a1.v[4]), "v"(b1.v[4]), "s"(a1.v[5]));
    asm("v_mad_u64_u32 %0, %1, %2, %3, %0\n\tv_mad_u64_u32 %0, %1, %4, %5, %0\n\tv_mad_u64_u32 %0, %1, %6, %7, %0\n\tv_mad_u64_u32 %0, %1, %8, 1, %0\n\tv_mad_i64_i32 %0, %1, %9, %10, %0\n\tv_mad_i64_i32 %0, %1, %11, %12, %0\n\tv_mad_i64_i32 %0, %1, %13, %14, %0\n\tv_mad_i64_i32 %0, %1, %15, %16, %0\n\tv_mad_i64_i32 %0, %1, %17, %18, %0"
        : "+&v"(nc), "=&s"(cc) : "v"(b1.v[3]), "s"(a1.v[6]), "v"(b1.v[2]), "s"(a1.v[7]), "v"(b1.v[1]), "s"(a1.v[8]), "v"(t.v[0]), "v"(m8), "s"(n1), "v"(m7), "s"(n2), "v"(m6), "s"(n3), "v"(m5), "s"(n4), "v"(m1), "s"(n8));
    col = nc;
    r.v[0] = (uint32_t)col & M29; col = (uint64_t)((int64_t)col >> 29);
    asm("v_mad_u64_u32 %0, %1, %2, %3, %0\n\tv_mad_u64_u32 %0, %1, %4, %5, %0\n\tv_mad_u64_u32 %0, %1, %6, %7, %0\n\tv_mad_u64_u32 %0, %1, %8, %9, %0\n\tv_mad_u64_u32 %0, %1, %10, %11, %0\n\tv_mad_u64_u32 %0, %1, %12, %13, %0\n\tv_mad_u64_u32 %0, %1, %14, %15, %0\n\tv_mad_u64_u32 %0, %1, %16, %17, %0\n\tv_mad_u64_u32 %0, %1, %18, %19, %0\n\tv_mad_u64_u32 %0, %1, %20, %21, %0\n\tv_mad_u64_u32 %0, %1, %22, %23, %0\n\tv_mad_u64_u32 %0, %1, %24, %25, %0\n\tv_mad_u64_u32 %0, %1, %26, %27, %0\n\tv_mad_u64_u32 %0, %1, %28, %29, %0"
        : "+&v"(col), "=&s"(cc) : "v"(b0.v[8]), "s"(a0.v[2]), "v"(b0.v[7]), "s"(a0.v[3]), "v"(b0.v[6]), "s"(a0.v[4]), "v"(b0.v[5]), "s"(a0.v[5]), "v"(b0.v[4]), "s"(a0.v[6]), "v"(b0.v[3]), "s"(a0.v[7]), "v"(b0.v[2]), "s"(a0.v[8]), "v"(b1.v[8]), "s"(a1.v[2]), "v"(b1.v[7]), "s"(a1.v[3]), "v"(b1.v[6]), "s"(a1.v[4]), "v"(b1.v[5]), "s"(a1.v[5]), "v"(b1.v[4]), "s"(a1.v[6]), "v"(b1.v[3]), "s"(a1.v[7]), "v"(b1.v[2]), "s"(a1.v[8]));
    asm("v_mad_u64_u32 %0, %1, %2, 1, %0\n\tv_mad_i64_i32 %0, %1, %3, %4, %0\n\tv_mad_i64_i32 %0, %1, %5, %6, %0\n\tv_mad_i64_i32 %0, %1, %7, %8, %0\n\tv_mad_i64_i32 %0, %1, %9, %10, %0"
        : "+&v"(col), "=&s"(cc) : "v"(t.v[1]), "v"(m8), "s"(n2), "v"(m7), "s"(n3), "v"(m6), "s"(n4), "v"(m2), "s"(n8));
    r.v[1] = (uint32_t)col & M29; col = (uint64_t)((int64_t)col >> 29);
    asm("v_mad_u64_u32 %0, %1, %2, %3, %0\n\tv_mad_u64_u32 %0, %1, %4, %5, %0\n\tv_mad_u64_u32 %0, %1, %6, %7, %0\n\tv_mad_u64_u32 %0, %1, %8, %9, %0\n\tv_mad_u64_u32 %0, %1, %10, %11, %0\n\tv_mad_u64_u32 %0, %1, %12, %13, %0\n\tv_mad_u64_u32 %0, %1, %14, %15, %0\n\tv_mad_u64_u32 %0, %1, %16, %17, %0\n\tv_mad_u64_u32 %0, %1, %18, %19, %0\n\tv_mad_u64_u32 %0, %1, %20, %21, %0\n\tv_mad_u64_u32 %0, %1, %22, %23, %0\n\tv_mad_u64_u32 %0, %1, %24, %25, %0\n\tv_mad_u64_u32 %0, %1, %26, 1, %0\n\tv_mad_i64_i32 %0, %1, %27, %28, %0"
        : "+&v"(col), "=&s"(cc) : "v"(b0.v[8]), "s"(a0.v[3]), "v"(b0.v[7]), "s"(a0.v[4]), "v"(b0.v[6]), "s"(a0.v[5]), "v"(b0.v[5]), "s"(a0.v[6]), "v"(b0.v[4]), "s"(a0.v[7]), "v"(b0.v[3]), "s"(a0.v[8]), "v"(b1.v[8]), "s"(a1.v[3]), "v"(b1.v[7]), "s"(a1.v[4]), "v"(b1.v[6]), "s"(a1.v[5]), "v"(b1.v[5]), "s"(a1.v[6]), "v"(b1.v[4]), "s"(a1.v[7]), "v"(b1.v[3]), "s"(a1.v[8]), "v"(t.v[2]), "v"(m8), "s"(n3));
    asm("v_mad_i64_i32 %0, %1, %2, %3, %0\n\tv_mad_i64_i32 %0, %1, %4, %5, %0"
        : "+&v"(col), "=&s"(cc) : "v"(m7), "s"(n4), "v"(m3), "s"(n8));
    r.v[2] = (uint32_t)col & M29; col = (uint64_t)((int64_t)col >> 29);
    asm("v_mad_u64_u32 %0, %1, %2, %3, %0\n\tv_mad_u64_u32 %0, %1, %4, %5, %0\n\tv_mad_u64_u32 %0, %1, %6, %7, %0\n\tv_mad_u64_u32 %0, %1, %8, %9, %0\n\tv_mad_u64_u32 %0, %1, %10, %11, %0\n\tv_mad_u64_u32 %0, %1, %12, %13, %0\n\tv_mad_u64_u32 %0, %1, %14, %15, %0\n\tv_mad_u64_u32 %0, %1, %16, %17, %0\n\tv_mad_u64_u32 %0, %1, %18, %19, %0\n\tv_mad_u64_u32 %0, %1, %20, %21, %0\n\tv_mad_u64_u32 %0, %1, %22, 1, %0\n\tv_mad_i64_i32 %0, %1, %23, %24, %0\n\tv_mad_i64_i32 %0, %1, %25, %26, %0"
        : "+&v"(col), "=&s"(cc) : "v"(b0.v[8]), "s"(a0.v[4]), "v"(b0.v[7]), "s"(a0.v[5]), "v"(b0.v[6]), "s"(a0.v[6]), "v"(b0.v[5]), "s"(a0.v[7]), "v"(b0.v[4]), "s"(a0.v[8]), "v"(b1.v[8]), "s"(a1.v[4]), "v"(b1.v[7]), "s"(a1.v[5]), "v"(b1.v[6]), "s"(a1.v[6]), "v"(b1.v[5]), "s"(a1.v[7]), "v"(b1.v[4]), "s"(a1.v[8]), "v"(t.v[3]), "v"(m8), "s"(n4), "v"(m4), "s"(n8));
    r.v[3] = (uint32_t)col & M29; col = (uint64_t)((int64_t)col >> 29);
    asm("v_mad_u64_u32 %0, %1, %2, %3, %0\n\tv_mad_u64_u32 %0, %1, %4, %5, %0\n\tv_mad_u64_u32 %0, %1, %6, %7, %0\n\tv_mad_u64_u32 %0, %1, %8, %9, %0\n\tv_mad_u64_u32 %0, %1, %10, %11, %0\n\tv_mad_u64_u32 %0, %1, %12, %13, %0\n\tv_mad_u64_u32 %0, %1, %14, %15, %0\n\tv_mad_u64_u32 %0, %1, %16, %17, %0\n\tv_mad_u64_u32 %0, %1, %18, 1, %0\n\tv_mad_i64_i32 %0, %1, %19, %20, %0"
        : "+&v"(col), "=&s"(cc) : "v"(b0.v[8]), "s"(a0.v[5]), "v"(b0.v[7]), "s"(a0.v[6]), "v"(b0.v[6]), "s"(a0.v[7]), "v"(b0.v[5]), "s"(a0.v[8]), "v"(b1.v[8]), "s"(a1.v[5]), "v"(b1.v[7]), "s"(a1.v[6]), "v"(b1.v[6]), "s"(a1.v[7]), "v"(b1.v[5]), "s"(a1.v[8]), "v"(t.v[4]), "v"(m5), "s"(n8));
    r.v[4] = (uint32_t)col & M29; col = (uint64_t)((int64_t)col >> 29);
    asm("v_mad_u64_u32 %0, %1, %2, %3, %0\n\tv_mad_u64_u32 %0, %1, %4, %5, %0\n\tv_mad_u64_u32 %0, %1, %6, %7, %0\n\tv_mad_u64_u32 %0, %1, %8, %9, %0\n\tv_mad_u64_u32 %0, %1, %10, %11, %0\n\tv_mad_u64_u32 %0, %1, %12, %13, %0\n\tv_mad_u64_u32 %0, %1, %14, 1, %0\n\tv_mad_i64_i32 %0, %1, %15, %16, %0"
        : "+&v"(col), "=&s"(cc) : "v"(b0.v[8]), "s"(a0.v[6]), "v"(b0.v[7]), "s"(a0.v[7]), "v"(b0.v[6]), "s"(a0.v[8]), "v"(b1.v[8]), "s"(a1.v[6]), "v"(b1.v[7]), "s"(a1.v[7]), "v"(b1.v[6]), "s"(a1.v[8]), "v"(t.v[5]), "v"(m6), "s"(n8));
    r.v[5] = (uint32_t)col & M29; col = (uint64_t)((int64_t)col >> 29);
    asm("v_mad_u64_u32 %0, %1, %2, %3, %0\n\tv_mad_u64_u32 %0, %1, %4, %5, %0\n\tv_mad_u64_u32 %0, %1, %6, %7, %0\n\tv_mad_u64_u32 %0, %1, %8, %9, %0\n\tv_mad_u64_u32 %0, %1, %10, 1, %0\n\tv_mad_i64_i32 %0, %1, %11, %12, %0"
        : "+&v"(col), "=&s"(cc) : "v"(b0.v[8]), "s"(a0.v[7]), "v"(b0.v[7]), "s"(a0.v[8]), "v"(b1.v[8]), "s"(a1.v[7]), "v"(b1.v[7]), "s"(a1.v[8]), "v"(t.v[6]), "v"(m7), "s"(n8));
    r.v[6] = (uint32_t)col & M29; col = (uint64_t)((int64_t)col >> 29);
    asm("v_mad_u64_u32 %0, %1, %2, %3, %0\n\tv_mad_u64_u32 %0, %1, %4, %5, %0\n\tv_mad_u64_u32 %0, %1, %6, 1, %0\n\tv_mad_i64_i32 %0, %1, %7, %8, %0"
        : "+&v"(col), "=&s"(cc) : "v"(b0.v[8]), "s"(a0.v[8]), "v"(b1.v[8]), "s"(a1.v[8]), "v"(t.v[7]), "v"(m8), "s"(n8));
    r.v[7] = (uint32_t)col & M29; col = (uint64_t)((int64_t)col >> 29);
    r.v[8] = (uint32_t)col + t.v[8];
    return r;
}
#endif

}
```

mina_bridge_amd/csrc/sponge.cuh:

```cuda
#pragma once
#include "groupmap.cuh"
#include "fp29.cuh"

namespace mb {

struct BpolyShape { uint32_t k, lb, hb, batch; };

template <int F>
__global__ void bpoly_tables_kernel(BpolyShape sh, FieldK fk, const uint32_t *__restrict__ chals ,
                                    const uint32_t *__restrict__ weights ,
                                    fe_t *__restrict__ ltab, fe_t *__restrict__ htab) { mb_wave_prio<1>();
    const uint32_t nl = 1u << sh.lb, nh = 1u << sh.hb, per = nl + nh;
    size_t gid = (size_t)blockIdx.x * blockDim.x + threadIdx.x;
    if (gid >= (size_t)sh.batch * per) return;
    uint32_t b = (uint32_t)(gid / per), e = (uint32_t)(gid % per);
    const uint32_t *cb = chals + (size_t)b * sh.k * 8;
    fe_t acc; uint32_t bits, base;
    if (e < nl) { bits = e; base = 0; acc = fk.one; }
    else {
        bits = e - nl; base = sh.lb;
        if (weights) { fe_t w; for (int i = 0; i < 8; ++i) w.v[i] = weights[(size_t)b * 8 + i]; acc = fe_to_mont<F>(w, fk.r2); }
        else acc = fk.one;
    }
    for (uint32_t q = 0; bits; ++q, bits >>= 1) {
// ... 61 lines not shown
}

template <int F>
__global__ void bpoly_eval_kernel(uint32_t k, uint32_t npoints, FieldK fk, const uint32_t *__restrict__ chals,
                                  const uint32_t *__restrict__ xs, uint32_t *__restrict__ out_words) {
    uint32_t p = blockIdx.x * blockDim.x + threadIdx.x;
    if (p >= npoints) return;
    fe_t x; for (int i = 0; i < 8; ++i) x.v[i] = xs[(size_t)p * 8 + i];
    fe_t pw = fe_to_mont<F>(x, fk.r2), r = fk.one;
    for (int i = (int)k - 1; i >= 0; --i) {
        fe_t c; for (int q = 0; q < 8; ++q) c.v[q] = chals[(size_t)i * 8 + q];
        r = fe_mul<F>(r, fe_add<F>(fk.one, fe_mul<F>(fe_to_mont<F>(c, fk.r2), pw)));
        pw = fe_sqr<F>(pw);
    }
    r = fe_from_mont<F>(r);
    for (int i = 0; i < 8; ++i) out_words[(size_t)p * 8 + i] = r.v[i];
}

struct PoseidonParams { fe_t mds[3][3]; fe_t rc[55][3]; };
struct PoseidonParams29 { fe29_t mds[3][3]; fe29_t rc[55][3]; fe29_t enter , leave ;
                          fe29_t rc2[55][3];
                          fe29_t zero;
                          fe29_t absorb;
                          uint32_t pad[1]; };
static_assert(sizeof(PoseidonParams29) % 16 == 0, "PoseidonParams29 is read with 16-byte loads");
__host__ __device__ static inline const PoseidonParams29 *pparams29_of(const PoseidonParams *pp) { return reinterpret_cast<const PoseidonParams29 *>(pp + 1); }
struct PoseidonRow1 { fe29_t a[2]; fe29_t rc; };
struct PoseidonRows1 { PoseidonRow1 row[54][3];
                       fe29_t last[3][3]; fe29_t last_rc[3];
                       uint32_t ok;
                       uint32_t pad[1]; };
static_assert(sizeof(PoseidonRows1) % 16 == 0, "PoseidonRows1 is read with 16-byte loads");
__host__ __device__ static inline const PoseidonRows1 *prows1_of(const PoseidonParams *pp) { return reinterpret_cast<const PoseidonRows1 *>(pparams29_of(pp) + 1); }

template <int F>
__device__ __forceinline__ void poseidon_permute(fe_t s[3], const PoseidonParams *__restrict__ pp) {
#pragma unroll 1
    for (int r = 0; r < 55; ++r) {
        fe_t t[3];
#pragma unroll
        for (int i = 0; i < 3; ++i) {
            fe_t x2 = fe_sqr<F>(s[i]);
            fe_t x4 = fe_sqr<F>(x2);
            t[i] = fe_mul<F>(fe_mul<F>(x4, x2), s[i]);
        }
#pragma unroll
        for (int i = 0; i < 3; ++i) {
            s[i] = fe_add<F>(fe_dot3<F>(pp->mds[i][0], t[0], pp->mds[i][1], t[1], pp->mds[i][2], t[2]), pp->rc[r][i]);
        }
    }
}

template <int F>
__global__ void __launch_bounds__(256)
poseidon_permute_kernel(uint32_t n, FieldK fk, const PoseidonParams *__restrict__ pp, uint32_t *__restrict__ states) {
    uint32_t i = blockIdx.x * blockDim.x + threadIdx.x;
    if (i >= n) return;
    fe_t s[3];
    for (int j = 0; j < 3; ++j) { fe_t w; for (int q = 0; q < 8; ++q) w.v[q] = states[(size_t)i * 24 + j * 8 + q]; s[j] = fe_to_mont<F>(w, fk.r2); }
    poseidon_permute<F>(s, pp);
    for (int j = 0; j < 3; ++j) { fe_t w = fe_from_mont<F>(s[j]); for (int q = 0; q < 8; ++q) states[(size_t)i * 24 + j * 8 + q] = w.v[q]; }
}

#if defined(__HIPCC__)
__device__ __forceinline__ fe_t pair_swap(const fe_t &a) {
    fe_t r = a;
// ... 84 lines not shown
template <int F>
__device__ __forceinline__ void poseidon_rounds_one(fe29_t x[3], const PoseidonRows1 *__restrict__ q1) {
#if defined(__HIP_DEVICE_COMPILE__)
#pragma unroll 1
    for (int r = 0; r < 54; ++r) {
        const PoseidonRow1 *__restrict__ rw = q1->row[r];
        fe29_t t[3];
#pragma unroll
        for (int i = 0; i < 3; ++i) {
            const fe29_t x2 = fe29_sqr_sg<F>(x[i]);
            const fe29_t x4 = fe29_sqr_sg<F>(x2);
            t[i] = fe29_mul_sg<F>(fe29_mul_sg<F>(x4, x2), x[i]);
        }
#pragma unroll
        for (int i = 0; i < 3; ++i) x[i] = fe29_row1_sg<F>(t[i], rw[i].a[0], t[i == 2 ? 0 : i + 1], rw[i].a[1], t[i == 0 ? 2 : i - 1], rw[i].rc);
    }
    fe29_t t[3];
#pragma unroll
    for (int i = 0; i < 3; ++i) {
        const fe29_t x2 = fe29_sqr_sg<F>(x[i]);
        const fe29_t x4 = fe29_sqr_sg<F>(x2);
        t[i] = fe29_mul_sg<F>(fe29_mul_sg<F>(x4, x2), x[i]);
    }
#pragma unroll
    for (int i = 0; i < 3; ++i) x[i] = fe29_dot3rc_sg<F>(q1->last[i][0], t[0], q1->last[i][1], t[1], q1->last[i][2], t[2], q1->last_rc[i]);
#else
    (void)x; (void)q1;
#endif
}
template <int F>
__device__ __forceinline__ void poseidon_permute_tri(fe_t &s, const PoseidonParams *__restrict__ pp) {
#if defined(__HIP_DEVICE_COMPILE__)
    const TriPos tp = tri_pos();
    const PoseidonParams29 *__restrict__ q = pparams29_of(pp);
    fe29_t x = fe29_mul_asm<F>(fe29_from_words(s), q->enter);
    poseidon_rounds_tri<F>(x, q, tp);
    s = fe_cond_sub_p<F>(fe29_to_words(fe29_mul_asm<F>(x, q->leave)));
#else
    (void)s; (void)pp;
#endif
}
template <int F>
__device__ __forceinline__ void poseidon_permute_hex(fe_t &s, const PoseidonParams *__restrict__ pp) {
#if defined(__HIP_DEVICE_COMPILE__)
    const uint32_t o = threadIdx.x & 15u, qd = o >> 2, c = o & 3u, e = qd < 3 ? qd : 2u, col = c < 3 ? c : 2u;
    const bool odd = c & 1u;
    const PoseidonParams29 *__restrict__ q = pparams29_of(pp);
    const fe29_t m = q->mds[e][col];
#define MB_QUAD29(NAME, CTRL) auto NAME = [](const fe29_t &a) { fe29_t r; _Pragma("unroll") for (int i = 0; i < L29; ++i) r.v[i] = (uint32_t)__builtin_amdgcn_mov_dpp((int)a.v[i], CTRL, 0xf, 0xf, true); return r; }
    MB_QUAD29(swap29, 0xB1);
    MB_QUAD29(rot1, 0x09);
    MB_QUAD29(rot2, 0x52);
#undef MB_QUAD29
    const int src = (int)(((threadIdx.x & 63u) & ~15u) | (col << 2));
    fe29_t x = fe29_mul_asm<F>(fe29_from_words(s), q->enter);
    const fe29_t *rcp = c == 0 ? &q->rc2[0][e] : &q->zero;
    const size_t rcs = c == 0 ? 3 : 0;
#pragma unroll 1
    for (int r = 0; r < 55; ++r) {
        const fe29_t x2 = fe29_sqr_sg<F>(x);
        const fe29_t y = fe29_mul_sg<F>(x2, odd ? x : x2);
        const fe29_t t = fe29_mul_sg<F>(y, swap29(y));
        fe29_t tc;
#pragma unroll
        for (int i = 0; i < L29; ++i) tc.v[i] = (uint32_t)__shfl((int)t.v[i], src, 64);
        const fe29_t pr = fe29_mulrc_sg<F>(m, tc, rcp[rcs * r]);
        x = fe29_add3(pr, rot1(pr), rot2(pr));
    }
    s = fe_cond_sub_p<F>(fe29_to_words(fe29_mul_asm<F>(x, q->leave)));
// ... 240 lines not shown
```

mina_bridge_amd/lib.py:

```python
from __future__ import annotations

import ctypes
import os

import numpy as np

HERE = os.path.dirname(os.path.abspath(__file__))
LIB_PATH = os.path.join(HERE, "libminaverify.so")

FIELD_FP, FIELD_FQ = 0, 1
CURVE_PALLAS, CURVE_VESTA = 0, 1

EXPORTS = [
    "mina_ctx_create", "mina_ctx_destroy", "mina_last_error", "mina_ctx_synchronize", "mina_ctx_stream", "mina_ctx_pin_lane", "mina_ctx_set_pipeline", "mina_prof_enable", "mina_prof_read",
    "mina_dev_malloc", "mina_dev_free", "mina_dev_upload", "mina_dev_download",
    "mina_srs_create", "mina_srs_split_table", "mina_srs_load", "mina_srs_depth", "mina_srs_get_g", "mina_srs_get_h", "mina_srs_lagrange_basis", "mina_public_input_commitment", "mina_public_input_commitment_batch", "mina_combined_inner_product", "mina_srs_serialize",
    "mina_msm", "mina_msm_srs", "mina_msm_srs_range", "mina_msm_srs_multi", "mina_msm_srs_dev",
    "mina_b_poly", "mina_b_poly_coefficients", "mina_b_poly_fold", "mina_b_poly_fold_dev",
    "mina_poseidon_set_params", "mina_poseidon_params_parse", "mina_poseidon_load_params", "mina_poseidon_load_params_file", "mina_poseidon_permute", "mina_poseidon_permute_dev", "mina_poseidon_hash",
    "mina_challenge_to_field", "mina_fq_sponge_run", "mina_to_group", "mina_merkle_roots", "mina_merkle_verify_batch",
    "mina_field_mul", "mina_field_inv", "mina_field_sqrt", "mina_selftest_group_law", "mina_selftest_fe29", "mina_selftest_fe32",
    "mina_accumulator_check_batch", "mina_accumulator_check_dev", "mina_accumulator_check_multi_dev", "mina_accumulator_check_multi", "mina_ipa_batch_check",
    "mina_consensus_project_window", "mina_consensus_relative_min_window_density", "mina_consensus_is_short_range",
    "mina_protocol_state_pack", "mina_protocol_state_hash_batch", "mina_protocol_state_hash_bytes",
# ... 160 lines not shown
        ("acc_rho", ctypes.c_void_p),
    ]

    POINTER_FIELDS = ("state_records", "state_nfields", "expected_hashes", "precheck", "public_inputs", "sponge_state", "sponge_pos", "cip", "lr",
                      "delta", "sg", "z1", "z2", "evalpoints", "evalscale", "polyscale", "comms", "rand_base", "sg_rand_base", "acc_prechallenges",
                      "acc_sg", "acc_rho")


class VerifierIndex(ctypes.Structure):
    _fields_ = [("log2_domain", ctypes.c_uint32), ("zk_rows", ctypes.c_uint32), ("perm_alpha_offset", ctypes.c_uint32), ("shifts", ctypes.c_void_p),
                ("sigma_comm", ctypes.c_void_p), ("coefficients_comm", ctypes.c_void_p), ("selector_comm", ctypes.c_void_p), ("constant_term", ctypes.c_void_p),
                ("constant_term_len", ctypes.c_size_t)]


class KimchiProofs(ctypes.Structure):
    _fields_ = [("batch", ctypes.c_size_t), ("n_prev", ctypes.c_uint32), ("npub", ctypes.c_uint32), ("public_inputs", ctypes.c_void_p), ("prev_chals", ctypes.c_void_p),
                ("prev_comms", ctypes.c_void_p), ("w_comm", ctypes.c_void_p), ("z_comm", ctypes.c_void_p), ("t_comm", ctypes.c_void_p), ("evals", ctypes.c_void_p),
                ("ft_eval1", ctypes.c_void_p), ("statements", ctypes.c_void_p), ("prev_prechallenges", ctypes.c_void_p)]
    POINTER_FIELDS = ("public_inputs", "prev_chals", "prev_comms", "w_comm", "z_comm", "t_comm", "evals", "ft_eval1", "prev_prechallenges")


class PicklesStatements(ctypes.Structure):
    POINTER_FIELDS = ("plonk", "bulletproof_challenges", "step_old_challenges", "step_comms", "wrap_old_challenges", "wrap_sg", "sponge_digest", "prev_evals",
                      "prev_public_input", "prev_ft_eval1", "app_state", "misc")
    _fields_ = [("n_old", ctypes.c_uint32), ("n_evals", ctypes.c_uint32)] + [(n, ctypes.c_void_p) for n in POINTER_FIELDS]

    def strides(self):
        return dict(zip(self.POINTER_FIELDS, (64, 256, self.n_old * 256, self.n_old * 64, 480, 64, 32, self.n_evals * 64, 64, 32, 32, 32)))

FE29_IN_OPERANDS, FE29_OUT_RESULTS = 8, 4
FE29_IN_WORDS, FE29_OUT_WORDS = FE29_IN_OPERANDS * 9 + 1, FE29_OUT_RESULTS * 9 + 1
FE29_FLAG_NEG, FE29_FLAG_OK, FE29_FLAG_INF = 1, 1, 2
FE29_OPS = {"MUL_ASM": 0, "SQR_ASM": 1, "DOT2_ASM": 2, "DOT3_ASM": 3, "SQR_HI_ASM": 4, "MUL_HI_ASM": 5, "MUL_LZ": 6, "SQR_LZ": 7, "MUL_HI_LZ": 8, "MULRC_LZ": 9, "DOT2RC_LZ": 10,
            "DOT3RC_LZ": 11, "MUL_SG": 12, "SQR_SG": 13, "MUL_HI_SG": 14, "SQR_HI_SG": 15, "MULRC_SG": 16, "DOT2RC_SG": 17, "DOT3RC_SG": 18, "ROW1_SG": 19,
            "SUB_KP_ONE": 32, "KP_MINUS_NEG_Y": 33, "KP_MINUS_SUB_X1": 34, "KP_MINUS_SUB_Y1": 35, "KP_MINUS_G_U1": 36, "KP_MINUS_G_S1": 37, "KP_MINUS_A_2B_X3_SUB": 38,
            "KP_MINUS_A_2B_G_X3_SUB": 39, "ADD_KP_MINUS_SUB_X3": 40, "ADD_KP_MINUS_G_SUB_X3": 41, "ADD": 42, "ADD3": 43, "WORDS": 44, "IS_MULTIPLE_OF_P": 45, "LEAVE": 46,
            "ADD_AFFINE": 64, "ADD_AFFINE_TWIN": 65, "XYZZ_ADD": 66, "XYZZ_LEAVE": 67}
FE32_IN_OPERANDS, FE32_OUT_RESULTS = 8, 4
FE32_IN_WORDS, FE32_OUT_WORDS = FE32_IN_OPERANDS * 8 + 1, FE32_OUT_RESULTS * 8 + 1
FE32_FLAG_TRUE, FE32_FLAG_LANES_AGREE = 1, 2
FE32_OPS = {"COND_SUB_P": 0, "ADD": 1, "SUB": 2, "NEG": 3, "DBL": 4, "MUL": 5, "SQR": 6, "DOT2": 7, "DOT3": 8, "TO_MONT": 9, "FROM_MONT": 10, "INV": 11, "SQRT": 12,
            "WORDS_CANONICAL": 13, "DBL_AFFINE": 32, "XYZZ_DBL": 33, "ADD_AFFINE": 34, "XYZZ_ADD": 35, "XYZZ_DBL_QUAD": 36, "XYZZ_ADD_QUAD": 37}


class KimchiBatchOut(ctypes.Structure):
    _fields_ = [("sponge_state", ctypes.c_void_p), ("sponge_pos", ctypes.c_void_p), ("cip", ctypes.c_void_p), ("evalpoints", ctypes.c_void_p), ("polyscale", ctypes.c_void_p),
                ("evalscale", ctypes.c_void_p), ("comms", ctypes.c_void_p), ("ft_eval0", ctypes.c_void_p), ("malformed", ctypes.c_void_p)]


CHECK_FORMAT, CHECK_LEDGER, CHECK_CHAIN, CHECK_CONSENSUS, CHECK_ACCUMULATOR, CHECK_KIMCHI, CHECK_ACCOUNT_ABI, CHECK_MERKLE = 1, 2, 4, 8, 16, 32, 64, 128
VERIFY_ALLOW_MISSING_KIMCHI, VERIFY_ALLOW_UNBOUND_STATEMENT, VERIFY_ALLOW_SURROGATE = 1, 2, 4
VERIFY_DEDUP_STATES = 8
VERIFY_ACCOUNT_ON_DEVICE = 32
VERIFY_PACK_ON_DEVICE = 16


def _bytes_arg(b):
    a = _u8(b) if len(b) else np.zeros(1, np.uint8)
    return a, ctypes.c_size_t(len(b))


def verify_state(proof: bytes, pub: bytes) -> bool:
    lib = load_library()
    lib.mina_verify_state.restype = ctypes.c_bool
    p, pl = _bytes_arg(proof); q, ql = _bytes_arg(pub)
    return bool(lib.mina_verify_state(_p(p), pl, _p(q), ql))

# ... 934 lines not shown
```

Measured before the change: 280,800.

## Rescale Poseidon MDS per lane so 3-lane rounds use per-lane row constants

Adds a host-side precomputation (PoseidonRows3) that rescales the Poseidon state per element, using seventh roots of the MDS diagonal, so each lane's diagonal coefficient becomes one. Each round then needs only two cross-lane products plus a round constant, through a new per-lane row1 variant. The 3-lane cooperative permutation now uses these tables, and lane selection falls back from 3 to 8 lanes when the table cannot be built. This is meant to cut multiplications per round in the 3-lane sponge path, at the cost of a larger parameter blob, more involved setup, and reliance on a seventh root existing for every diagonal entry.

```diff
diff --git a/include/mina_verify.h b/include/mina_verify.h
--- a/include/mina_verify.h
+++ b/include/mina_verify.h
@@ -123,6 +123,7 @@
 #define MINA_FE29_DOT2RC_SG 17
 #define MINA_FE29_DOT3RC_SG 18
 #define MINA_FE29_ROW1_SG 19
+#define MINA_FE29_ROW1V_SG 21
 #define MINA_FE29_SUB_KP_ONE 32
 #define MINA_FE29_KP_MINUS_NEG_Y 33
 #define MINA_FE29_KP_MINUS_SUB_X1 34
diff --git a/mina_bridge_amd/csrc/api_account.hip b/mina_bridge_amd/csrc/api_account.hip
--- a/mina_bridge_amd/csrc/api_account.hip
+++ b/mina_bridge_amd/csrc/api_account.hip
@@ -46,7 +46,7 @@
     const PoseidonParams *pp = c->pparams[FIELD_FP].as<PoseidonParams>();
     const fe_t *salts = c->state_salts.as<fe_t>();
     ProfScope ps_(c, PS_STATE_HASH);
-    return with_lanes<16, 8, 3>(hash_lanes(c, n, n), [&](auto lanes) {
+    return with_lanes<16, 8, 3>(hash_lanes(c, n, n, tri_rows(c, FIELD_FP)), [&](auto lanes) {
         constexpr int LN = decltype(lanes)::value;
         mb::salted_hash_kernel<FIELD_FP, LN><<<cdiv(coop_threads<LN>(n), 256), 256, 0, c->L->stream>>>((uint32_t)n, c->fk[FIELD_FP], pp, salts, salt_idx, recs, nf, pa, sa, pb, sb, out);
         HIPC(hipGetLastError());
diff --git a/mina_bridge_amd/csrc/api_account_dev.hip b/mina_bridge_amd/csrc/api_account_dev.hip
--- a/mina_bridge_amd/csrc/api_account_dev.hip
+++ b/mina_bridge_amd/csrc/api_account_dev.hip
@@ -19,7 +19,7 @@
     const PoseidonParams *pp = c->pparams[FIELD_FP].as<PoseidonParams>();
     const fe_t *salts = c->state_salts.as<fe_t>();
     ProfScope ps_(c, PS_STATE_HASH);
-    return with_lanes<16, 8, 3>(hash_lanes(c, n, n * roles), [&](auto lanes) {
+    return with_lanes<16, 8, 3>(hash_lanes(c, n, n * roles, tri_rows(c, FIELD_FP)), [&](auto lanes) {
         constexpr int LN = decltype(lanes)::value;
         mb::acct_hash_kernel<FIELD_FP, LN><<<cdiv(coop_threads<LN>(n * roles), 256), 256, 0, c->L->stream>>>((uint32_t)n, roles, count_dev, c->fk[FIELD_FP], pp, salts, salt_idx, recs, nf, pa, sa,
                                                                                                            pb, sb, marks, pa_default, out_index, out);
@@ -104,7 +104,7 @@
                             W(w.h_uri) + n * 8, mw::ZK_SLOT_VK, nullptr, nullptr, W(w.zk_index), W(w.h_zkapp)))) return rc;
     if ((rc = acct_hash_dev(c, n, 1, nullptr, stage(w.salt_idx, mb::AS_ACCOUNT, 4), stage(w.records, mb::AS_ACCOUNT, REC_BYTES), stage(w.nfields, mb::AS_ACCOUNT, 4), W(w.h_zkapp), mb::AR_ZKAPP_HASH,
                             nullptr, 0, W(w.marks), defaults + 16, nullptr, W(w.h_account)))) return rc;
-    if ((rc = with_lanes<16, 8, 3>(merkle_lanes(c, n), [&](auto lanes) {
+    if ((rc = with_lanes<16, 8, 3>(merkle_lanes(c, n, tri_rows(c, FIELD_FP)), [&](auto lanes) {
             constexpr int LN = decltype(lanes)::value;
             mb::acct_fold_kernel<FIELD_FP, LN><<<cdiv(coop_threads<LN>(n), 256), 256, 0, L.stream>>>((uint32_t)n, c->fk[FIELD_FP], c->pparams[FIELD_FP].as<PoseidonParams>(),
                 c->merkle_salts[FIELD_FP].as<fe_t>(), W(w.h_account), W(w.siblings), d + w.dirs, W(w.depths), W(w.roots));
diff --git a/mina_bridge_amd/csrc/api_core.hip b/mina_bridge_amd/csrc/api_core.hip
--- a/mina_bridge_amd/csrc/api_core.hip
+++ b/mina_bridge_amd/csrc/api_core.hip
@@ -80,7 +80,7 @@
         if (a.srs_gen != b.srs_gen || a.lagrange_log2 != b.lagrange_log2 || (a.lagrange_host.empty() && !b.lagrange_host.empty())) { a.lagrange_host = b.lagrange_host; a.lagrange_log2 = b.lagrange_log2; a.srs_gen = b.srs_gen; }
         a.lagrange_table.alias(b.lagrange_table); a.lagrange_table_n = b.lagrange_table_n; a.lagrange_table_log2 = b.lagrange_table_log2;
         a.lagrange_digits.alias(b.lagrange_digits); a.lagrange_digits29.alias(b.lagrange_digits29); a.lagrange_digits_n = b.lagrange_digits_n;
-        v->pparams[i].alias(p->pparams[i]); v->have_pparams[i] = p->have_pparams[i]; v->pparams_surrogate[i] = p->pparams_surrogate[i]; v->pparams_rows1[i] = p->pparams_rows1[i];
+        v->pparams[i].alias(p->pparams[i]); v->have_pparams[i] = p->have_pparams[i]; v->pparams_surrogate[i] = p->pparams_surrogate[i]; v->pparams_rows1[i] = p->pparams_rows1[i]; v->pparams_rows3[i] = p->pparams_rows3[i];
         v->merkle_salts[i].alias(p->merkle_salts[i]); v->merkle_depth[i] = p->merkle_depth[i];
     }
     v->kimchi_index.alias(p->kimchi_index); v->kimchi_tokens.alias(p->kimchi_tokens); v->kimchi_literals.alias(p->kimchi_literals);
diff --git a/mina_bridge_amd/csrc/api_ipa.hip b/mina_bridge_amd/csrc/api_ipa.hip
--- a/mina_bridge_amd/csrc/api_ipa.hip
+++ b/mina_bridge_amd/csrc/api_ipa.hip
@@ -481,7 +481,7 @@
             if (!L.aux) { HIPC(hipStreamCreateWithFlags(&L.aux, hipStreamNonBlocking)); HIPC(hipEventCreateWithFlags(&L.ev_fork, hipEventDisableTiming)); HIPC(hipEventCreateWithFlags(&L.ev_join, hipEventDisableTiming)); }
             tg = L.aux;
         }
-        const int ln = transcript_lanes(c, batch, (size_t)tune.ipa_coop8_max);
+        const int ln = transcript_lanes(c, batch, (size_t)tune.ipa_coop8_max, tri_rows_both(c));
         auto prepare = [&](auto phase) {
             return with_lanes<16, 8, 3>(ln, [&](auto lanes) {
                 constexpr int LN = decltype(lanes)::value, PH = decltype(phase)::value;
@@ -635,7 +635,7 @@
     if ((rc = L.ipa_chals.ensure(batch * 8))) return rc;
     const PoseidonParams *pp = c->pparams[FB].as<PoseidonParams>();
     const int FS = scalar_field_of(curve);
-    if ((rc = with_lanes<8, 3>(sponge_batch_lanes(batch), [&](auto lanes) {
+    if ((rc = with_lanes<8, 3>(sponge_batch_lanes(batch, tri_rows_both(c)), [&](auto lanes) {
             constexpr int LN = decltype(lanes)::value;
             DISPATCH_CURVE(curve, {
                 mb::sponge_tape_kernel<C_, LN><<<cdiv(coop_threads<LN>(batch), 64), 64, 0, L.stream>>>((uint32_t)batch, (uint32_t)tape_len, (uint32_t)in_words, (uint32_t)out_words,
diff --git a/mina_bridge_amd/csrc/api_kimchi.hip b/mina_bridge_amd/csrc/api_kimchi.hip
--- a/mina_bridge_amd/csrc/api_kimchi.hip
+++ b/mina_bridge_amd/csrc/api_kimchi.hip
@@ -327,7 +327,7 @@
     const FieldK &kb = c->fk[FIELD_FP], &ks = c->fk[FIELD_FQ];
     mb::kimchi_rows_kernel<<<cdiv(batch * ncomms * 16, 256), 256, 0, L.stream>>>(B, n_prev, ix, in, out.comms);
     const uint32_t fq_roles = pf_digest ? 1u : 2u;
-    if ((rc = with_lanes<16, 8, 3>(transcript_lanes(c, batch, (size_t)mb_tune().kimchi_coop8_max), [&](auto lanes) {
+    if ((rc = with_lanes<16, 8, 3>(transcript_lanes(c, batch, (size_t)mb_tune().kimchi_coop8_max, tri_rows_both(c)), [&](auto lanes) {
             constexpr int LN = decltype(lanes)::value;
             mb::kimchi_fq_kernel<LN><<<fq_roles * coop_role_blocks<LN>(batch), 64, 0, L.stream>>>(B, n_prev, kb, ks, ppb, pps, ix, in, out, xf, d_bad, coop_role_blocks<LN>(batch), (const fe_t *)pf_digest, pf_stride);
             if (npub > 32 && npub <= 40) mb::kimchi_pub_kernel<10><<<cdiv(batch * 8, 64), 64, 0, L.stream>>>(B, npub, ks, ix, in, xf, d_bad);
diff --git a/mina_bridge_amd/csrc/api_pickles.hip b/mina_bridge_amd/csrc/api_pickles.hip
--- a/mina_bridge_amd/csrc/api_pickles.hip
+++ b/mina_bridge_amd/csrc/api_pickles.hip
@@ -464,7 +464,7 @@
     ProfScope ps_(c, PS_PICKLES);
     HIPC(hipMemsetD32Async((hipDeviceptr_t)d_ok, 1, batch, L.stream));
     mb::pickles_expand_kernel<<<cdiv(batch * (50 + 16 * in.n_old), 256), 256, 0, L.stream>>>(B, kp, kq, in, xe);
-    if ((rc = with_lanes<16, 8, 3>(transcript_lanes(c, batch, 1024), [&](auto lanes) {
+    if ((rc = with_lanes<16, 8, 3>(transcript_lanes(c, batch, 1024, tri_rows_both(c)), [&](auto lanes) {
             constexpr int LN = decltype(lanes)::value;
             mb::pickles_digest_kernel<LN><<<3 * coop_role_blocks<LN>(batch), 64, 0, L.stream>>>(B, kp, kq, ppp, ppq, ix, in, xe, d_ok, coop_role_blocks<LN>(batch));
             mb::pickles_tick_kernel<LN><<<cdiv(coop_threads<LN>(batch), 64), 64, 0, L.stream>>>(B, kp, ppp, in, xe, d_ok);
diff --git a/mina_bridge_amd/csrc/api_selftest.hip b/mina_bridge_amd/csrc/api_selftest.hip
--- a/mina_bridge_amd/csrc/api_selftest.hip
+++ b/mina_bridge_amd/csrc/api_selftest.hip
@@ -8,7 +8,7 @@
     X(MINA_FE29_MUL_ASM) X(MINA_FE29_SQR_ASM) X(MINA_FE29_DOT2_ASM) X(MINA_FE29_DOT3_ASM) X(MINA_FE29_SQR_HI_ASM) X(MINA_FE29_MUL_HI_ASM)                            \
     X(MINA_FE29_MUL_LZ) X(MINA_FE29_SQR_LZ) X(MINA_FE29_MUL_HI_LZ) X(MINA_FE29_MULRC_LZ) X(MINA_FE29_DOT2RC_LZ) X(MINA_FE29_DOT3RC_LZ)                               \
     X(MINA_FE29_MUL_SG) X(MINA_FE29_SQR_SG) X(MINA_FE29_MUL_HI_SG) X(MINA_FE29_SQR_HI_SG) X(MINA_FE29_MULRC_SG) X(MINA_FE29_DOT2RC_SG) X(MINA_FE29_DOT3RC_SG)        \
-    X(MINA_FE29_ROW1_SG)                                                                                                                                             \
+    X(MINA_FE29_ROW1_SG) X(MINA_FE29_ROW1V_SG)                                                                                                                       \
     X(MINA_FE29_SUB_KP_ONE) X(MINA_FE29_KP_MINUS_NEG_Y) X(MINA_FE29_KP_MINUS_SUB_X1) X(MINA_FE29_KP_MINUS_SUB_Y1) X(MINA_FE29_KP_MINUS_G_U1) X(MINA_FE29_KP_MINUS_G_S1) \
     X(MINA_FE29_KP_MINUS_A_2B_X3_SUB) X(MINA_FE29_KP_MINUS_A_2B_G_X3_SUB) X(MINA_FE29_ADD_KP_MINUS_SUB_X3) X(MINA_FE29_ADD_KP_MINUS_G_SUB_X3)                        \
     X(MINA_FE29_ADD) X(MINA_FE29_ADD3) X(MINA_FE29_WORDS) X(MINA_FE29_IS_MULTIPLE_OF_P) X(MINA_FE29_LEAVE)                                                           \
@@ -54,6 +54,7 @@
     else if constexpr (OP == MINA_FE29_DOT2RC_SG) o[0] = fe29_dot2rc_sg<F>(s[0], s[1], s[2], s[3], s[6]);
     else if constexpr (OP == MINA_FE29_DOT3RC_SG) o[0] = fe29_dot3rc_sg<F>(s[0], s[1], s[2], s[3], s[4], s[5], s[6]);
     else if constexpr (OP == MINA_FE29_ROW1_SG) o[0] = fe29_row1_sg<F>(s[7], s[0], s[1], s[2], s[3], s[6]);
+    else if constexpr (OP == MINA_FE29_ROW1V_SG) o[0] = fe29_row1_sg<F, FE29_PER_LANE>(s[7], s[0], s[1], s[2], s[3], s[6]);
     else if constexpr (OP == MINA_FE29_SUB_KP_ONE) o[0] = fe29_sub_kp<F, 1>(s[0], s[1]);
     else if constexpr (OP == MINA_FE29_KP_MINUS_NEG_Y) o[0] = fe29_kp_minus<F, EC29::NEG_Y_MULT>(s[0]);
     else if constexpr (OP == MINA_FE29_KP_MINUS_SUB_X1) o[0] = fe29_kp_minus<F, EC29::SUB_X1_MULT>(s[0]);
diff --git a/mina_bridge_amd/csrc/api_sponge.hip b/mina_bridge_amd/csrc/api_sponge.hip
--- a/mina_bridge_amd/csrc/api_sponge.hip
+++ b/mina_bridge_amd/csrc/api_sponge.hip
@@ -137,15 +137,54 @@
     return true;
 }
 
+template <int F> static bool poseidon_rows3(const PoseidonParams &pp, const FieldK &k, const fe_t &two5, const fe_t &two522, PoseidonRows3 &out) {
+    for (int i = 0; i < 3; ++i) if (fe_is_zero(pp.mds[i][i])) return false;
+    fe_t e7 = fe_zero(); bool have_e7 = false;
+    uint32_t n[8]; { uint64_t cy = 1; for (int i = 0; i < 8; ++i) { cy += k.pm2.v[i]; n[i] = (uint32_t)cy; cy >>= 32; } if (cy) return false; }
+    for (uint32_t j = 1; j <= 6 && !have_e7; ++j) {
+        uint32_t t[9]; uint64_t cy = 1;
+        for (int i = 0; i < 8; ++i) { cy += (uint64_t)n[i] * j; t[i] = (uint32_t)cy; cy >>= 32; }
+        t[8] = (uint32_t)cy;
+        uint32_t qd[9]; uint64_t rem = 0;
+        for (int i = 8; i >= 0; --i) { const uint64_t cur = (rem << 32) | t[i]; qd[i] = (uint32_t)(cur / 7); rem = cur % 7; }
+        if (rem == 0 && qd[8] == 0) { for (int i = 0; i < 8; ++i) e7.v[i] = qd[i]; have_e7 = true; }
+    }
+    if (!have_e7) return false;
+    auto pow7 = [&](const fe_t &a) { const fe_t a2 = fe_mul<F>(a, a), a4 = fe_mul<F>(a2, a2); return fe_mul<F>(fe_mul<F>(a4, a2), a); };
+    auto to29 = [&](const fe_t &a, const fe_t &scale) { return fe29_from_words(fe_mul<F>(a, scale)); };
+    fe_t dn[3] = {k.one, k.one, k.one};
+    for (int r = 54; r >= 0; --r) {
+        fe_t d[3], d7inv[3];
+        for (int j = 0; j < 3; ++j) {
+            const fe_t arg = fe_mul<F>(dn[j], pp.mds[j][j]);
+            d[j] = fe_pow<F>(arg, e7, k.one);
+            if (!fe_eq(pow7(d[j]), arg)) return false;
+            d7inv[j] = fe_inv<F>(arg, k);
+        }
+        for (int i = 0; i < 3; ++i) {
+            fe_t a[3];
+            for (int j = 0; j < 3; ++j) a[j] = fe_mul<F>(fe_mul<F>(dn[i], pp.mds[i][j]), d7inv[j]);
+            if (!fe_eq(a[i], k.one)) return false;
+            PoseidonRow3 &w = out.row[r][i];
+            w.a[0] = to29(a[i == 2 ? 0 : i + 1], two5); w.a[1] = to29(a[i == 0 ? 2 : i - 1], two5); w.rc = to29(fe_mul<F>(dn[i], pp.rc[r][i]), two522);
+        }
+        for (int j = 0; j < 3; ++j) dn[j] = d[j];
+    }
+    for (int e = 0; e < 3; ++e) out.enter[e] = fe29_from_words(fe_mul<F>(fe_mul<F>(two5, two5), dn[e]));
+    out.ok = 1;
+    return true;
+}
+
 bool mb_params_are_surrogate(int field, const uint8_t *params);
 extern "C" int mina_poseidon_set_params(mina_ctx *c, int field, const uint8_t *params) {
     if (!c || !params) return fail(MINA_ERR_ARG, "null argument");
     if (bad_field(field)) return fail(MINA_ERR_ARG, "bad field");
     HIPC(hipSetDevice(c->device));
     c->use_lane0();
-    struct { PoseidonParams pp; PoseidonParams29 q; PoseidonRows1 q1; } both;
+    struct { PoseidonParams pp; PoseidonParams29 q; PoseidonRows1 q1; PoseidonRows3 q3; } both;
     PoseidonParams &pp = both.pp;
-    static_assert(sizeof(both) == sizeof(PoseidonParams) + sizeof(PoseidonParams29) + sizeof(PoseidonRows1), "PoseidonParams29 sits right behind PoseidonParams, PoseidonRows1 behind it");
+    static_assert(sizeof(both) == sizeof(PoseidonParams) + sizeof(PoseidonParams29) + sizeof(PoseidonRows1) + sizeof(PoseidonRows3), "PoseidonParams29 sits right behind PoseidonParams, PoseidonRows1 behind it, PoseidonRows3 last");
+    static_assert((sizeof(PoseidonParams) + sizeof(PoseidonParams29) + sizeof(PoseidonRows1)) % 16 == 0, "PoseidonRows3 starts on a 16-byte boundary");
     memset(&both, 0, sizeof both);
     DISPATCH_FIELD(field, {
         params_to_mont<F_>(params, c->fk[F_], pp);
@@ -159,6 +198,7 @@
         both.q.absorb = fe29_from_words(two522);
         both.q.leave = fe29_from_words(k.one);
         if (!poseidon_rows1<F_>(pp, k, two5, two522, both.q1)) memset(&both.q1, 0, sizeof both.q1);
+        if (!poseidon_rows3<F_>(pp, k, two5, two522, both.q3)) memset(&both.q3, 0, sizeof both.q3);
     });
     int rc;
     if ((rc = c->pparams[field].ensure(sizeof both))) return rc;
@@ -166,6 +206,7 @@
     HIPC(hipStreamSynchronize(c->L->stream));
     c->have_pparams[field] = true;
     c->pparams_rows1[field] = both.q1.ok != 0;
+    c->pparams_rows3[field] = both.q3.ok != 0;
     c->pparams_surrogate[field] = mb_params_are_surrogate(field, params);
     c->merkle_depth[field] = 0;
     if (field == FIELD_FP) { c->have_state_salts = false; c->have_acct_defaults = false; }
@@ -210,7 +251,7 @@
     int rc;
     if ((rc = h2d(c, c->L->tmp_a, inputs, n * len * 32))) return rc;
     if ((rc = c->L->tmp_c.ensure(n * 32))) return rc;
-    if ((rc = with_lanes<8, 3>(sponge_batch_lanes(n), [&](auto lanes) {
+    if ((rc = with_lanes<8, 3>(sponge_batch_lanes(n, tri_rows(c, field)), [&](auto lanes) {
             constexpr int LN = decltype(lanes)::value;
             DISPATCH_FIELD(field, { poseidon_hash_coop_kernel<F_, LN><<<cdiv(coop_threads<LN>(n), 256), 256, 0, c->L->stream>>>((uint32_t)n, (uint32_t)len, c->fk[F_], c->pparams[field].as<PoseidonParams>(), c->L->tmp_a.as<uint32_t>(), c->L->tmp_c.as<uint32_t>()); });
             return MINA_OK;
@@ -250,7 +291,7 @@
 }
 
 int mb_merkle_fold_dev(mina_ctx *c, int field, size_t n, uint32_t depth, const uint32_t *d_leaves, const uint32_t *d_sib, const uint8_t *d_dirs, uint32_t *d_roots) {
-    return with_lanes<16, 8, 3>(merkle_lanes(c, n), [&](auto lanes) {
+    return with_lanes<16, 8, 3>(merkle_lanes(c, n, tri_rows(c, field)), [&](auto lanes) {
         constexpr int LN = decltype(lanes)::value;
         DISPATCH_FIELD(field, {
             merkle_fold_coop_kernel<F_, LN><<<cdiv(coop_threads<LN>(n), 256), 256, 0, c->L->stream>>>((uint32_t)n, depth, c->fk[F_], c->pparams[field].as<PoseidonParams>(),
diff --git a/mina_bridge_amd/csrc/ctx.h b/mina_bridge_amd/csrc/ctx.h
--- a/mina_bridge_amd/csrc/ctx.h
+++ b/mina_bridge_amd/csrc/ctx.h
@@ -144,6 +144,7 @@
     void *step_host = nullptr; void (*step_host_free)(void *) = nullptr;
     bool pparams_surrogate[2] = {false, false};
     bool pparams_rows1[2] = {false, false};
+    bool pparams_rows3[2] = {false, false};
     DevBuf state_salts; bool have_state_salts = false;
     bool is_view = false;
     bool state_dedup = false;
@@ -194,15 +195,18 @@
 }
 static inline size_t hash_piece_states(const mina_ctx *c, size_t leg_states, uint32_t piece_waves) { return (size_t)piece_waves * (hash_one_lane(c, leg_states) ? 64u : 21u); }
 
-static inline int hash_lanes(const mina_ctx *c, size_t proofs, size_t sponges) { return use_coop16(c, proofs) ? 16 : (use_coop8(c, sponges) ? 8 : 3); }
+static inline bool tri_rows(const mina_ctx *c, int field) { return c->pparams_rows3[field]; }
+static inline bool tri_rows_both(const mina_ctx *c) { return c->pparams_rows3[0] && c->pparams_rows3[1]; }
+static inline int tri_or_oct(int lanes, bool rows3) { return lanes == 3 && !rows3 ? 8 : lanes; }
+static inline int hash_lanes(const mina_ctx *c, size_t proofs, size_t sponges, bool rows3) { return tri_or_oct(use_coop16(c, proofs) ? 16 : (use_coop8(c, sponges) ? 8 : 3), rows3); }
 static inline int pstate_hash_lanes(const mina_ctx *c, size_t n, size_t leg_states) {
-    return hash_one_lane(c, leg_states) ? 1 : hash_lanes(c, (n + MINA_STATES_PER_PROOF - 1) / MINA_STATES_PER_PROOF, n);
-}
-static inline int transcript_lanes(const mina_ctx *c, size_t batch, size_t per_call_limit) {
-    return use_coop16(c, batch) ? 16 : (use_coop8_transcripts(c, batch, per_call_limit) ? 8 : 3);
-}
-static inline int sponge_batch_lanes(size_t n) { return n <= COOP8_MAX_GROUPS ? 8 : 3; }
-static inline int merkle_lanes(const mina_ctx *c, size_t paths) { return use_coop16(c, paths) ? 16 : sponge_batch_lanes(paths); }
+    return hash_one_lane(c, leg_states) ? 1 : hash_lanes(c, (n + MINA_STATES_PER_PROOF - 1) / MINA_STATES_PER_PROOF, n, true);
+}
+static inline int transcript_lanes(const mina_ctx *c, size_t batch, size_t per_call_limit, bool rows3) {
+    return tri_or_oct(use_coop16(c, batch) ? 16 : (use_coop8_transcripts(c, batch, per_call_limit) ? 8 : 3), rows3);
+}
+static inline int sponge_batch_lanes(size_t n, bool rows3) { return tri_or_oct(n <= COOP8_MAX_GROUPS ? 8 : 3, rows3); }
+static inline int merkle_lanes(const mina_ctx *c, size_t paths, bool rows3) { return use_coop16(c, paths) ? 16 : sponge_batch_lanes(paths, rows3); }
 
 enum : uint32_t { MB_JOB_LEGS = 1, MB_JOB_FINISH = 2, MB_JOB_ALL = 3 };
 struct StateJobCarry { uint32_t *ipa_v = nullptr, *acc_v = nullptr, *kimchi_bad = nullptr; const uint32_t *stmt_ok = nullptr; };
diff --git a/mina_bridge_amd/csrc/fp29.cuh b/mina_bridge_amd/csrc/fp29.cuh
--- a/mina_bridge_amd/csrc/fp29.cuh
+++ b/mina_bridge_amd/csrc/fp29.cuh
@@ -73,6 +73,7 @@
     static constexpr uint32_t LANES8_STATE_MILLI_P = 4100;
     static constexpr uint32_t LANES16_STATE_MILLI_P = 6100;
     static constexpr uint32_t LANES1_STATE_MILLI_P = 6300;
+    static constexpr uint32_t LANES3N_STATE_MILLI_P = 4200;
 };
 
 #if defined(__HIP_DEVICE_COMPILE__)
@@ -1821,6 +1822,91 @@
     r.v[8] = (uint32_t)col + t.v[8];
     return r;
 }
+static constexpr int FE29_PER_LANE = 1;
+template <int F, int OPERANDS> __device__ __forceinline__ fe29_t fe29_row1_sg(const fe29_t &t, const fe29_t &a0, const fe29_t &b0, const fe29_t &a1, const fe29_t &b1, const fe29_t &c) {
+    static_assert(OPERANDS == FE29_PER_LANE, "fe29_row1_sg<F> takes wave-uniform constants, fe29_row1_sg<F, FE29_PER_LANE> per-lane ones");
+    uint64_t col, nc, cc; fe29_t r;
+    uint32_t m0, m1, m2, m3, m4, m5, m6, m7, m8;
+    const int32_t n1 = -(int32_t)P29<F>::L1, n2 = -(int32_t)P29<F>::L2, n3 = -(int32_t)P29<F>::L3, n4 = -(int32_t)P29<F>::L4, n8 = -(int32_t)P29<F>::L8;
+    asm("v_mad_u64_u32 %0, %1, %2, %3, 0\n\tv_mad_u64_u32 %0, %1, %4, %5, %0\n\tv_mad_u64_u32 %0, %1, %6, 1, %0"
+        : "=&v"(col), "=&s"(cc) : "v"(a0.v[0]), "v"(b0.v[0]), "v"(a1.v[0]), "v"(b1.v[0]), "v"(c.v[0]));
+    m0 = (uint32_t)col;
+    asm("v_mad_i64_i32 %0, %1, %2, -1, %3\n\tv_ashrrev_i64 %0, 29, %0\n\tv_mad_u64_u32 %0, %1, %4, %5, %0\n\tv_mad_u64_u32 %0, %1, %6, %7, %0\n\tv_mad_u64_u32 %0, %1, %8, %9, %0\n\tv_mad_u64_u32 %0, %1, %10, %11, %0\n\tv_mad_u64_u32 %0, %1, %12, 1, %0\n\tv_mad_i64_i32 %0, %1, %13, %14, %0"
+        : "=&v"(nc), "=&s"(cc) : "v"(m0), "v"(col), "v"(a0.v[0]), "v"(b0.v[1]), "v"(a0.v[1]), "v"(b0.v[0]), "v"(a1.v[0]), "v"(b1.v[1]), "v"(a1.v[1]), "v"(b1.v[0]), "v"(c.v[1]), "v"(m0), "s"(n1));
+    col = nc;
+    m1 = (uint32_t)col;
+    asm("v_mad_i64_i32 %0, %1, %2, -1, %3\n\tv_ashrrev_i64 %0, 29, %0\n\tv_mad_u64_u32 %0, %1, %4, %5, %0\n\tv_mad_u64_u32 %0, %1, %6, %7, %0\n\tv_mad_u64_u32 %0, %1, %8, %9, %0\n\tv_mad_u64_u32 %0, %1, %10, %11, %0\n\tv_mad_u64_u32 %0, %1, %12, %13, %0\n\tv_mad_u64_u32 %0, %1, %14, %15, %0\n\tv_mad_u64_u32 %0, %1, %16, 1, %0\n\tv_mad_i64_i32 %0, %1, %17, %18, %0\n\tv_mad_i64_i32 %0, %1, %19, %20, %0"
+        : "=&v"(nc), "=&s"(cc) : "v"(m1), "v"(col), "v"(a0.v[0]), "v"(b0.v[2]), "v"(a0.v[1]), "v"(b0.v[1]), "v"(a0.v[2]), "v"(b0.v[0]), "v"(a1.v[0]), "v"(b1.v[2]), "v"(a1.v[1]), "v"(b1.v[1]), "v"(a1.v[2]), "v"(b1.v[0]), "v"(c.v[2]), "v"(m1), "s"(n1), "v"(m0), "s"(n2));
+    col = nc;
+    m2 = (uint32_t)col;
+    asm("v_mad_i64_i32 %0, %1, %2, -1, %3\n\tv_ashrrev_i64 %0, 29, %0\n\tv_mad_u64_u32 %0, %1, %4, %5, %0\n\tv_mad_u64_u32 %0, %1, %6, %7, %0\n\tv_mad_u64_u32 %0, %1, %8, %9, %0\n\tv_mad_u64_u32 %0, %1, %10, %11, %0\n\tv_mad_u64_u32 %0, %1, %12, %13, %0\n\tv_mad_u64_u32 %0, %1, %14, %15, %0\n\tv_mad_u64_u32 %0, %1, %16, %17, %0\n\tv_mad_u64_u32 %0, %1, %18, %19, %0\n\tv_mad_u64_u32 %0, %1, %20, 1, %0\n\tv_mad_i64_i32 %0, %1, %21, %22, %0\n\tv_mad_i64_i32 %0, %1, %23, %24, %0\n\tv_mad_i64_i32 %0, %1, %25, %26, %0"
+        : "=&v"(nc), "=&s"(cc) : "v"(m2), "v"(col), "v"(a0.v[0]), "v"(b0.v[3]), "v"(a0.v[1]), "v"(b0.v[2]), "v"(a0.v[2]), "v"(b0.v[1]), "v"(a0.v[3]), "v"(b0.v[0]), "v"(a1.v[0]), "v"(b1.v[3]), "v"(a1.v[1]), "v"(b1.v[2]), "v"(a1.v[2]), "v"(b1.v[1]), "v"(a1.v[3]), "v"(b1.v[0]), "v"(c.v[3]), "v"(m2), "s"(n1), "v"(m1), "s"(n2), "v"(m0), "s"(n3));
+    col = nc;
+    m3 = (uint32_t)col;
+    asm("v_mad_i64_i32 %0, %1, %2, -1, %3\n\tv_ashrrev_i64 %0, 29, %0\n\tv_mad_u64_u32 %0, %1, %4, %5, %0\n\tv_mad_u64_u32 %0, %1, %6, %7, %0\n\tv_mad_u64_u32 %0, %1, %8, %9, %0\n\tv_mad_u64_u32 %0, %1, %10, %11, %0\n\tv_mad_u64_u32 %0, %1, %12, %13, %0\n\tv_mad_u64_u32 %0, %1, %14, %15, %0\n\tv_mad_u64_u32 %0, %1, %16, %17, %0\n\tv_mad_u64_u32 %0, %1, %18, %19, %0\n\tv_mad_u64_u32 %0, %1, %20, %21, %0\n\tv_mad_u64_u32 %0, %1, %22, %23, %0\n\tv_mad_u64_u32 %0, %1, %24, 1, %0\n\tv_mad_i64_i32 %0, %1, %25, %26, %0\n\tv_mad_i64_i32 %0, %1, %27, %28, %0"
+        : "=&v"(nc), "=&s"(cc) : "v"(m3), "v"(col), "v"(a0.v[0]), "v"(b0.v[4]), "v"(a0.v[1]), "v"(b0.v[3]), "v"(a0.v[2]), "v"(b0.v[2]), "v"(a0.v[3]), "v"(b0.v[1]), "v"(a0.v[4]), "v"(b0.v[0]), "v"(a1.v[0]), "v"(b1.v[4]), "v"(a1.v[1]), "v"(b1.v[3]), "v"(a1.v[2]), "v"(b1.v[2]), "v"(a1.v[3]), "v"(b1.v[1]), "v"(a1.v[4]), "v"(b1.v[0]), "v"(c.v[4]), "v"(m3), "s"(n1), "v"(m2), "s"(n2));
+    asm("v_mad_i64_i32 %0, %1, %2, %3, %0\n\tv_mad_i64_i32 %0, %1, %4, %5, %0"
+        : "+&v"(nc), "=&s"(cc) : "v"(m1), "s"(n3), "v"(m0), "s"(n4));
+    col = nc;
+    m4 = (uint32_t)col;
+    asm("v_mad_i64_i32 %0, %1, %2, -1, %3\n\tv_ashrrev_i64 %0, 29, %0\n\tv_mad_u64_u32 %0, %1, %4, %5, %0\n\tv_mad_u64_u32 %0, %1, %6, %7, %0\n\tv_mad_u64_u32 %0, %1, %8, %9, %0\n\tv_mad_u64_u32 %0, %1, %10, %11, %0\n\tv_mad_u64_u32 %0, %1, %12, %13, %0\n\tv_mad_u64_u32 %0, %1, %14, %15, %0\n\tv_mad_u64_u32 %0, %1, %16, %17, %0\n\tv_mad_u64_u32 %0, %1, %18, %19, %0\n\tv_mad_u64_u32 %0, %1, %20, %21, %0\n\tv_mad_u64_u32 %0, %1, %22, %23, %0\n\tv_mad_u64_u32 %0, %1, %24, %25, %0\n\tv_mad_u64_u32 %0, %1, %26, %27, %0\n\tv_mad_u64_u32 %0, %1, %28, 1, %0"
+        : "=&v"(nc), "=&s"(cc) : "v"(m4), "v"(col), "v"(a0.v[0]), "v"(b0.v[5]), "v"(a0.v[1]), "v"(b0.v[4]), "v"(a0.v[2]), "v"(b0.v[3]), "v"(a0.v[3]), "v"(b0.v[2]), "v"(a0.v[4]), "v"(b0.v[1]), "v"(a0.v[5]), "v"(b0.v[0]), "v"(a1.v[0]), "v"(b1.v[5]), "v"(a1.v[1]), "v"(b1.v[4]), "v"(a1.v[2]), "v"(b1.v[3]), "v"(a1.v[3]), "v"(b1.v[2]), "v"(a1.v[4]), "v"(b1.v[1]), "v"(a1.v[5]), "v"(b1.v[0]), "v"(c.v[5]));
+    asm("v_mad_i64_i32 %0, %1, %2, %3, %0\n\tv_mad_i64_i32 %0, %1, %4, %5, %0\n\tv_mad_i64_i32 %0, %1, %6, %7, %0\n\tv_mad_i64_i32 %0, %1, %8, %9, %0"
+        : "+&v"(nc), "=&s"(cc) : "v"(m4), "s"(n1), "v"(m3), "s"(n2), "v"(m2), "s"(n3), "v"(m1), "s"(n4));
+    col = nc;
+    m5 = (uint32_t)col;
+    asm("v_mad_i64_i32 %0, %1, %2, -1, %3\n\tv_ashrrev_i64 %0, 29, %0\n\tv_mad_u64_u32 %0, %1, %4, %5, %0\n\tv_mad_u64_u32 %0, %1, %6, %7, %0\n\tv_mad_u64_u32 %0, %1, %8, %9, %0\n\tv_mad_u64_u32 %0, %1, %10, %11, %0\n\tv_mad_u64_u32 %0, %1, %12, %13, %0\n\tv_mad_u64_u32 %0, %1, %14, %15, %0\n\tv_mad_u64_u32 %0, %1, %16, %17, %0\n\tv_mad_u64_u32 %0, %1, %18, %19, %0\n\tv_mad_u64_u32 %0, %1, %20, %21, %0\n\tv_mad_u64_u32 %0, %1, %22, %23, %0\n\tv_mad_u64_u32 %0, %1, %24, %25, %0\n\tv_mad_u64_u32 %0, %1, %26, %27, %0\n\tv_mad_u64_u32 %0, %1, %28, %29, %0"
+        : "=&v"(nc), "=&s"(cc) : "v"(m5), "v"(col), "v"(a0.v[0]), "v"(b0.v[6]), "v"(a0.v[1]), "v"(b0.v[5]), "v"(a0.v[2]), "v"(b0.v[4]), "v"(a0.v[3]), "v"(b0.v[3]), "v"(a0.v[4]), "v"(b0.v[2]), "v"(a0.v[5]), "v"(b0.v[1]), "v"(a0.v[6]), "v"(b0.v[0]), "v"(a1.v[0]), "v"(b1.v[6]), "v"(a1.v[1]), "v"(b1.v[5]), "v"(a1.v[2]), "v"(b1.v[4]), "v"(a1.v[3]), "v"(b1.v[3]), "v"(a1.v[4]), "v"(b1.v[2]), "v"(a1.v[5]), "v"(b1.v[1]));
+    asm("v_mad_u64_u32 %0, %1, %2, %3, %0\n\tv_mad_u64_u32 %0, %1, %4, 1, %0\n\tv_mad_i64_i32 %0, %1, %5, %6, %0\n\tv_mad_i64_i32 %0, %1, %7, %8, %0\n\tv_mad_i64_i32 %0, %1, %9, %10, %0\n\tv_mad_i64_i32 %0, %1, %11, %12, %0"
+        : "+&v"(nc), "=&s"(cc) : "v"(a1.v[6]), "v"(b1.v[0]), "v"(c.v[6]), "v"(m5), "s"(n1), "v"(m4), "s"(n2), "v"(m3), "s"(n3), "v"(m2), "s"(n4));
+    col = nc;
+    m6 = (uint32_t)col;
+    asm("v_mad_i64_i32 %0, %1, %2, -1, %3\n\tv_ashrrev_i64 %0, 29, %0\n\tv_mad_u64_u32 %0, %1, %4, %5, %0\n\tv_mad_u64_u32 %0, %1, %6, %7, %0\n\tv_mad_u64_u32 %0, %1, %8, %9, %0\n\tv_mad_u64_u32 %0, %1, %10, %11, %0\n\tv_mad_u64_u32 %0, %1, %12, %13, %0\n\tv_mad_u64_u32 %0, %1, %14, %15, %0\n\tv_mad_u64_u32 %0, %1, %16, %17, %0\n\tv_mad_u64_u32 %0, %1, %18, %19, %0\n\tv_mad_u64_u32 %0, %1, %20, %21, %0\n\tv_mad_u64_u32 %0, %1, %22, %23, %0\n\tv_mad_u64_u32 %0, %1, %24, %25, %0\n\tv_mad_u64_u32 %0, %1, %26, %27, %0\n\tv_mad_u64_u32 %0, %1, %28, %29, %0"
+        : "=&v"(nc), "=&s"(cc) : "v"(m6), "v"(col), "v"(a0.v[0]), "v"(b0.v[7]), "v"(a0.v[1]), "v"(b0.v[6]), "v"(a0.v[2]), "v"(b0.v[5]), "v"(a0.v[3]), "v"(b0.v[4]), "v"(a0.v[4]), "v"(b0.v[3]), "v"(a0.v[5]), "v"(b0.v[2]), "v"(a0.v[6]), "v"(b0.v[1]), "v"(a0.v[7]), "v"(b0.v[0]), "v"(a1.v[0]), "v"(b1.v[7]), "v"(a1.v[1]), "v"(b1.v[6]), "v"(a1.v[2]), "v"(b1.v[5]), "v"(a1.v[3]), "v"(b1.v[4]), "v"(a1.v[4]), "v"(b1.v[3]));
+    asm("v_mad_u64_u32 %0, %1, %2, %3, %0\n\tv_mad_u64_u32 %0, %1, %4, %5, %0\n\tv_mad_u64_u32 %0, %1, %6, %7, %0\n\tv_mad_u64_u32 %0, %1, %8, 1, %0\n\tv_mad_i64_i32 %0, %1, %9, %10, %0\n\tv_mad_i64_i32 %0, %1, %11, %12, %0\n\tv_mad_i64_i32 %0, %1, %13, %14, %0\n\tv_mad_i64_i32 %0, %1, %15, %16, %0"
+        : "+&v"(nc), "=&s"(cc) : "v"(a1.v[5]), "v"(b1.v[2]), "v"(a1.v[6]), "v"(b1.v[1]), "v"(a1.v[7]), "v"(b1.v[0]), "v"(c.v[7]), "v"(m6), "s"(n1), "v"(m5), "s"(n2), "v"(m4), "s"(n3), "v"(m3), "s"(n4));
+    col = nc;
+    m7 = (uint32_t)col;
+    asm("v_mad_i64_i32 %0, %1, %2, -1, %3\n\tv_ashrrev_i64 %0, 29, %0\n\tv_mad_u64_u32 %0, %1, %4, %5, %0\n\tv_mad_u64_u32 %0, %1, %6, %7, %0\n\tv_mad_u64_u32 %0, %1, %8, %9, %0\n\tv_mad_u64_u32 %0, %1, %10, %11, %0\n\tv_mad_u64_u32 %0, %1, %12, %13, %0\n\tv_mad_u64_u32 %0, %1, %14, %15, %0\n\tv_mad_u64_u32 %0, %1, %16, %17, %0\n\tv_mad_u64_u32 %0, %1, %18, %19, %0\n\tv_mad_u64_u32 %0, %1, %20, %21, %0\n\tv_mad_u64_u32 %0, %1, %22, %23, %0\n\tv_mad_u64_u32 %0, %1, %24, %25, %0\n\tv_mad_u64_u32 %0, %1, %26, %27, %0\n\tv_mad_u64_u32 %0, %1, %28, %29, %0"
+        : "=&v"(nc), "=&s"(cc) : "v"(m7), "v"(col), "v"(a0.v[0]), "v"(b0.v[8]), "v"(a0.v[1]), "v"(b0.v[7]), "v"(a0.v[2]), "v"(b0.v[6]), "v"(a0.v[3]), "v"(b0.v[5]), "v"(a0.v[4]), "v"(b0.v[4]), "v"(a0.v[5]), "v"(b0.v[3]), "v"(a0.v[6]), "v"(b0.v[2]), "v"(a0.v[7]), "v"(b0.v[1]), "v"(a0.v[8]), "v"(b0.v[0]), "v"(a1.v[0]), "v"(b1.v[8]), "v"(a1.v[1]), "v"(b1.v[7]), "v"(a1.v[2]), "v"(b1.v[6]), "v"(a1.v[3]), "v"(b1.v[5]));
+    asm("v_mad_u64_u32 %0, %1, %2, %3, %0\n\tv_mad_u64_u32 %0, %1, %4, %5, %0\n\tv_mad_u64_u32 %0, %1, %6, %7, %0\n\tv_mad_u64_u32 %0, %1, %8, %9, %0\n\tv_mad_u64_u32 %0, %1, %10, %11, %0\n\tv_mad_u64_u32 %0, %1, %12, 1, %0\n\tv_mad_i64_i32 %0, %1, %13, %14, %0\n\tv_mad_i64_i32 %0, %1, %15, %16, %0\n\tv_mad_i64_i32 %0, %1, %17, %18, %0\n\tv_mad_i64_i32 %0, %1, %19, %20, %0\n\tv_mad_i64_i32 %0, %1, %21, %22, %0"
+        : "+&v"(nc), "=&s"(cc) : "v"(a1.v[4]), "v"(b1.v[4]), "v"(a1.v[5]), "v"(b1.v[3]), "v"(a1.v[6]), "v"(b1.v[2]), "v"(a1.v[7]), "v"(b1.v[1]), "v"(a1.v[8]), "v"(b1.v[0]), "v"(c.v[8]), "v"(m7), "s"(n1), "v"(m6), "s"(n2), "v"(m5), "s"(n3), "v"(m4), "s"(n4), "v"(m0), "s"(n8));
+    col = nc;
+    m8 = ((uint32_t)col & M29) | 0xC0000000u;
+    asm("v_mad_i64_i32 %0, %1, %2, -1, %3\n\tv_ashrrev_i64 %0, 29, %0\n\tv_mad_u64_u32 %0, %1, %4, %5, %0\n\tv_mad_u64_u32 %0, %1, %6, %7, %0\n\tv_mad_u64_u32 %0, %1, %8, %9, %0\n\tv_mad_u64_u32 %0, %1, %10, %11, %0\n\tv_mad_u64_u32 %0, %1, %12, %13, %0\n\tv_mad_u64_u32 %0, %1, %14, %15, %0\n\tv_mad_u64_u32 %0, %1, %16, %17, %0\n\tv_mad_u64_u32 %0, %1, %18, %19, %0\n\tv_mad_u64_u32 %0, %1, %20, %21, %0\n\tv_mad_u64_u32 %0, %1, %22, %23, %0\n\tv_mad_u64_u32 %0, %1, %24, %25, %0\n\tv_mad_u64_u32 %0, %1, %26, %27, %0\n\tv_mad_u64_u32 %0, %1, %28, %29, %0"
+        : "=&v"(nc), "=&s"(cc) : "v"(m8), "v"(col), "v"(a0.v[1]), "v"(b0.v[8]), "v"(a0.v[2]), "v"(b0.v[7]), "v"(a0.v[3]), "v"(b0.v[6]), "v"(a0.v[4]), "v"(b0.v[5]), "v"(a0.v[5]), "v"(b0.v[4]), "v"(a0.v[6]), "v"(b0.v[3]), "v"(a0.v[7]), "v"(b0.v[2]), "v"(a0.v[8]), "v"(b0.v[1]), "v"(a1.v[1]), "v"(b1.v[8]), "v"(a1.v[2]), "v"(b1.v[7]), "v"(a1.v[3]), "v"(b1.v[6]), "v"(a1.v[4]), "v"(b1.v[5]), "v"(a1.v[5]), "v"(b1.v[4]));
+    asm("v_mad_u64_u32 %0, %1, %2, %3, %0\n\tv_mad_u64_u32 %0, %1, %4, %5, %0\n\tv_mad_u64_u32 %0, %1, %6, %7, %0\n\tv_mad_u64_u32 %0, %1, %8, 1, %0\n\tv_mad_i64_i32 %0, %1, %9, %10, %0\n\tv_mad_i64_i32 %0, %1, %11, %12, %0\n\tv_mad_i64_i32 %0, %1, %13, %14, %0\n\tv_mad_i64_i32 %0, %1, %15, %16, %0\n\tv_mad_i64_i32 %0, %1, %17, %18, %0"
+        : "+&v"(nc), "=&s"(cc) : "v"(a1.v[6]), "v"(b1.v[3]), "v"(a1.v[7]), "v"(b1.v[2]), "v"(a1.v[8]), "v"(b1.v[1]), "v"(t.v[0]), "v"(m8), "s"(n1), "v"(m7), "s"(n2), "v"(m6), "s"(n3), "v"(m5), "s"(n4), "v"(m1), "s"(n8));
+    col = nc;
+    r.v[0] = (uint32_t)col & M29; col = (uint64_t)((int64_t)col >> 29);
+    asm("v_mad_u64_u32 %0, %1, %2, %3, %0\n\tv_mad_u64_u32 %0, %1, %4, %5, %0\n\tv_mad_u64_u32 %0, %1, %6, %7, %0\n\tv_mad_u64_u32 %0, %1, %8, %9, %0\n\tv_mad_u64_u32 %0, %1, %10, %11, %0\n\tv_mad_u64_u32 %0, %1, %12, %13, %0\n\tv_mad_u64_u32 %0, %1, %14, %15, %0\n\tv_mad_u64_u32 %0, %1, %16, %17, %0\n\tv_mad_u64_u32 %0, %1, %18, %19, %0\n\tv_mad_u64_u32 %0, %1, %20, %21, %0\n\tv_mad_u64_u32 %0, %1, %22, %23, %0\n\tv_mad_u64_u32 %0, %1, %24, %25, %0\n\tv_mad_u64_u32 %0, %1, %26, %27, %0\n\tv_mad_u64_u32 %0, %1, %28, %29, %0"
+        : "+&v"(col), "=&s"(cc) : "v"(a0.v[2]), "v"(b0.v[8]), "v"(a0.v[3]), "v"(b0.v[7]), "v"(a0.v[4]), "v"(b0.v[6]), "v"(a0.v[5]), "v"(b0.v[5]), "v"(a0.v[6]), "v"(b0.v[4]), "v"(a0.v[7]), "v"(b0.v[3]), "v"(a0.v[8]), "v"(b0.v[2]), "v"(a1.v[2]), "v"(b1.v[8]), "v"(a1.v[3]), "v"(b1.v[7]), "v"(a1.v[4]), "v"(b1.v[6]), "v"(a1.v[5]), "v"(b1.v[5]), "v"(a1.v[6]), "v"(b1.v[4]), "v"(a1.v[7]), "v"(b1.v[3]), "v"(a1.v[8]), "v"(b1.v[2]));
+    asm("v_mad_u64_u32 %0, %1, %2, 1, %0\n\tv_mad_i64_i32 %0, %1, %3, %4, %0\n\tv_mad_i64_i32 %0, %1, %5, %6, %0\n\tv_mad_i64_i32 %0, %1, %7, %8, %0\n\tv_mad_i64_i32 %0, %1, %9, %10, %0"
+        : "+&v"(col), "=&s"(cc) : "v"(t.v[1]), "v"(m8), "s"(n2), "v"(m7), "s"(n3), "v"(m6), "s"(n4), "v"(m2), "s"(n8));
+    r.v[1] = (uint32_t)col & M29; col = (uint64_t)((int64_t)col >> 29);
+    asm("v_mad_u64_u32 %0, %1, %2, %3, %0\n\tv_mad_u64_u32 %0, %1, %4, %5, %0\n\tv_mad_u64_u32 %0, %1, %6, %7, %0\n\tv_mad_u64_u32 %0, %1, %8, %9, %0\n\tv_mad_u64_u32 %0, %1, %10, %11, %0\n\tv_mad_u64_u32 %0, %1, %12, %13, %0\n\tv_mad_u64_u32 %0, %1, %14, %15, %0\n\tv_mad_u64_u32 %0, %1, %16, %17, %0\n\tv_mad_u64_u32 %0, %1, %18, %19, %0\n\tv_mad_u64_u32 %0, %1, %20, %21, %0\n\tv_mad_u64_u32 %0, %1, %22, %23, %0\n\tv_mad_u64_u32 %0, %1, %24, %25, %0\n\tv_mad_u64_u32 %0, %1, %26, 1, %0\n\tv_mad_i64_i32 %0, %1, %27, %28, %0"
+        : "+&v"(col), "=&s"(cc) : "v"(a0.v[3]), "v"(b0.v[8]), "v"(a0.v[4]), "v"(b0.v[7]), "v"(a0.v[5]), "v"(b0.v[6]), "v"(a0.v[6]), "v"(b0.v[5]), "v"(a0.v[7]), "v"(b0.v[4]), "v"(a0.v[8]), "v"(b0.v[3]), "v"(a1.v[3]), "v"(b1.v[8]), "v"(a1.v[4]), "v"(b1.v[7]), "v"(a1.v[5]), "v"(b1.v[6]), "v"(a1.v[6]), "v"(b1.v[5]), "v"(a1.v[7]), "v"(b1.v[4]), "v"(a1.v[8]), "v"(b1.v[3]), "v"(t.v[2]), "v"(m8), "s"(n3));
+    asm("v_mad_i64_i32 %0, %1, %2, %3, %0\n\tv_mad_i64_i32 %0, %1, %4, %5, %0"
+        : "+&v"(col), "=&s"(cc) : "v"(m7), "s"(n4), "v"(m3), "s"(n8));
+    r.v[2] = (uint32_t)col & M29; col = (uint64_t)((int64_t)col >> 29);
+    asm("v_mad_u64_u32 %0, %1, %2, %3, %0\n\tv_mad_u64_u32 %0, %1, %4, %5, %0\n\tv_mad_u64_u32 %0, %1, %6, %7, %0\n\tv_mad_u64_u32 %0, %1, %8, %9, %0\n\tv_mad_u64_u32 %0, %1, %10, %11, %0\n\tv_mad_u64_u32 %0, %1, %12, %13, %0\n\tv_mad_u64_u32 %0, %1, %14, %15, %0\n\tv_mad_u64_u32 %0, %1, %16, %17, %0\n\tv_mad_u64_u32 %0, %1, %18, %19, %0\n\tv_mad_u64_u32 %0, %1, %20, %21, %0\n\tv_mad_u64_u32 %0, %1, %22, 1, %0\n\tv_mad_i64_i32 %0, %1, %23, %24, %0\n\tv_mad_i64_i32 %0, %1, %25, %26, %0"
+        : "+&v"(col), "=&s"(cc) : "v"(a0.v[4]), "v"(b0.v[8]), "v"(a0.v[5]), "v"(b0.v[7]), "v"(a0.v[6]), "v"(b0.v[6]), "v"(a0.v[7]), "v"(b0.v[5]), "v"(a0.v[8]), "v"(b0.v[4]), "v"(a1.v[4]), "v"(b1.v[8]), "v"(a1.v[5]), "v"(b1.v[7]), "v"(a1.v[6]), "v"(b1.v[6]), "v"(a1.v[7]), "v"(b1.v[5]), "v"(a1.v[8]), "v"(b1.v[4]), "v"(t.v[3]), "v"(m8), "s"(n4), "v"(m4), "s"(n8));
+    r.v[3] = (uint32_t)col & M29; col = (uint64_t)((int64_t)col >> 29);
+    asm("v_mad_u64_u32 %0, %1, %2, %3, %0\n\tv_mad_u64_u32 %0, %1, %4, %5, %0\n\tv_mad_u64_u32 %0, %1, %6, %7, %0\n\tv_mad_u64_u32 %0, %1, %8, %9, %0\n\tv_mad_u64_u32 %0, %1, %10, %11, %0\n\tv_mad_u64_u32 %0, %1, %12, %13, %0\n\tv_mad_u64_u32 %0, %1, %14, %15, %0\n\tv_mad_u64_u32 %0, %1, %16, %17, %0\n\tv_mad_u64_u32 %0, %1, %18, 1, %0\n\tv_mad_i64_i32 %0, %1, %19, %20, %0"
+        : "+&v"(col), "=&s"(cc) : "v"(a0.v[5]), "v"(b0.v[8]), "v"(a0.v[6]), "v"(b0.v[7]), "v"(a0.v[7]), "v"(b0.v[6]), "v"(a0.v[8]), "v"(b0.v[5]), "v"(a1.v[5]), "v"(b1.v[8]), "v"(a1.v[6]), "v"(b1.v[7]), "v"(a1.v[7]), "v"(b1.v[6]), "v"(a1.v[8]), "v"(b1.v[5]), "v"(t.v[4]), "v"(m5), "s"(n8));
+    r.v[4] = (uint32_t)col & M29; col = (uint64_t)((int64_t)col >> 29);
+    asm("v_mad_u64_u32 %0, %1, %2, %3, %0\n\tv_mad_u64_u32 %0, %1, %4, %5, %0\n\tv_mad_u64_u32 %0, %1, %6, %7, %0\n\tv_mad_u64_u32 %0, %1, %8, %9, %0\n\tv_mad_u64_u32 %0, %1, %10, %11, %0\n\tv_mad_u64_u32 %0, %1, %12, %13, %0\n\tv_mad_u64_u32 %0, %1, %14, 1, %0\n\tv_mad_i64_i32 %0, %1, %15, %16, %0"
+        : "+&v"(col), "=&s"(cc) : "v"(a0.v[6]), "v"(b0.v[8]), "v"(a0.v[7]), "v"(b0.v[7]), "v"(a0.v[8]), "v"(b0.v[6]), "v"(a1.v[6]), "v"(b1.v[8]), "v"(a1.v[7]), "v"(b1.v[7]), "v"(a1.v[8]), "v"(b1.v[6]), "v"(t.v[5]), "v"(m6), "s"(n8));
+    r.v[5] = (uint32_t)col & M29; col = (uint64_t)((int64_t)col >> 29);
+    asm("v_mad_u64_u32 %0, %1, %2, %3, %0\n\tv_mad_u64_u32 %0, %1, %4, %5, %0\n\tv_mad_u64_u32 %0, %1, %6, %7, %0\n\tv_mad_u64_u32 %0, %1, %8, %9, %0\n\tv_mad_u64_u32 %0, %1, %10, 1, %0\n\tv_mad_i64_i32 %0, %1, %11, %12, %0"
+        : "+&v"(col), "=&s"(cc) : "v"(a0.v[7]), "v"(b0.v[8]), "v"(a0.v[8]), "v"(b0.v[7]), "v"(a1.v[7]), "v"(b1.v[8]), "v"(a1.v[8]), "v"(b1.v[7]), "v"(t.v[6]), "v"(m7), "s"(n8));
+    r.v[6] = (uint32_t)col & M29; col = (uint64_t)((int64_t)col >> 29);
+    asm("v_mad_u64_u32 %0, %1, %2, %3, %0\n\tv_mad_u64_u32 %0, %1, %4, %5, %0\n\tv_mad_u64_u32 %0, %1, %6, 1, %0\n\tv_mad_i64_i32 %0, %1, %7, %8, %0"
+        : "+&v"(col), "=&s"(cc) : "v"(a0.v[8]), "v"(b0.v[8]), "v"(a1.v[8]), "v"(b1.v[8]), "v"(t.v[7]), "v"(m8), "s"(n8));
+    r.v[7] = (uint32_t)col & M29; col = (uint64_t)((int64_t)col >> 29);
+    r.v[8] = (uint32_t)col + t.v[8];
+    return r;
+}
 #endif
 
 }
diff --git a/mina_bridge_amd/csrc/sponge.cuh b/mina_bridge_amd/csrc/sponge.cuh
--- a/mina_bridge_amd/csrc/sponge.cuh
+++ b/mina_bridge_amd/csrc/sponge.cuh
@@ -117,6 +117,13 @@
                        uint32_t pad[1]; };
 static_assert(sizeof(PoseidonRows1) % 16 == 0, "PoseidonRows1 is read with 16-byte loads");
 __host__ __device__ static inline const PoseidonRows1 *prows1_of(const PoseidonParams *pp) { return reinterpret_cast<const PoseidonRows1 *>(pparams29_of(pp) + 1); }
+struct alignas(16) PoseidonRow3 { fe29_t a[2]; fe29_t rc; uint32_t pad; };
+struct PoseidonRows3 { PoseidonRow3 row[55][3];
+                       fe29_t enter[3];
+                       uint32_t ok;
+                     };
+static_assert(sizeof(PoseidonRow3) == 112 && sizeof(PoseidonRows3) % 16 == 0, "PoseidonRows3 is read with 16-byte loads");
+__host__ __device__ static inline const PoseidonRows3 *prows3_of(const PoseidonParams *pp) { return reinterpret_cast<const PoseidonRows3 *>(prows1_of(pp) + 1); }
 
 template <int F>
 __device__ __forceinline__ void poseidon_permute(fe_t s[3], const PoseidonParams *__restrict__ pp) {
@@ -267,9 +274,19 @@
 __device__ __forceinline__ void poseidon_permute_tri(fe_t &s, const PoseidonParams *__restrict__ pp) {
 #if defined(__HIP_DEVICE_COMPILE__)
     const TriPos tp = tri_pos();
+    const uint32_t en = tp.e == 2u ? 0u : tp.e + 1u, ep = tp.e == 0u ? 2u : tp.e - 1u;
+    const PoseidonRows3 *__restrict__ q3 = prows3_of(pp);
+    fe29_t x = fe29_mul_asm<F>(fe29_from_words(s), q3->enter[tp.e]);
+#pragma unroll 1
+    for (int r = 0; r < 55; ++r) {
+        const PoseidonRow3 rw = q3->row[r][tp.e];
+        const fe29_t x2 = fe29_sqr_sg<F>(x);
+        const fe29_t x4 = fe29_sqr_sg<F>(x2);
+        const fe29_t t = fe29_mul_sg<F>(fe29_mul_sg<F>(x4, x2), x);
+        const fe29_t tn = tri_bcast29(t, tp.base + en), tq = tri_bcast29(t, tp.base + ep);
+        x = fe29_row1_sg<F, FE29_PER_LANE>(t, rw.a[0], tn, rw.a[1], tq, rw.rc);
+    }
     const PoseidonParams29 *__restrict__ q = pparams29_of(pp);
-    fe29_t x = fe29_mul_asm<F>(fe29_from_words(s), q->enter);
-    poseidon_rounds_tri<F>(x, q, tp);
     s = fe_cond_sub_p<F>(fe29_to_words(fe29_mul_asm<F>(x, q->leave)));
 #else
     (void)s; (void)pp;
diff --git a/mina_bridge_amd/lib.py b/mina_bridge_amd/lib.py
--- a/mina_bridge_amd/lib.py
+++ b/mina_bridge_amd/lib.py
@@ -216,7 +216,7 @@
 FE29_IN_WORDS, FE29_OUT_WORDS = FE29_IN_OPERANDS * 9 + 1, FE29_OUT_RESULTS * 9 + 1
 FE29_FLAG_NEG, FE29_FLAG_OK, FE29_FLAG_INF = 1, 1, 2
 FE29_OPS = {"MUL_ASM": 0, "SQR_ASM": 1, "DOT2_ASM": 2, "DOT3_ASM": 3, "SQR_HI_ASM": 4, "MUL_HI_ASM": 5, "MUL_LZ": 6, "SQR_LZ": 7, "MUL_HI_LZ": 8, "MULRC_LZ": 9, "DOT2RC_LZ": 10,
-            "DOT3RC_LZ": 11, "MUL_SG": 12, "SQR_SG": 13, "MUL_HI_SG": 14, "SQR_HI_SG": 15, "MULRC_SG": 16, "DOT2RC_SG": 17, "DOT3RC_SG": 18, "ROW1_SG": 19,
+            "DOT3RC_LZ": 11, "MUL_SG": 12, "SQR_SG": 13, "MUL_HI_SG": 14, "SQR_HI_SG": 15, "MULRC_SG": 16, "DOT2RC_SG": 17, "DOT3RC_SG": 18, "ROW1_SG": 19, "ROW1V_SG": 21,
             "SUB_KP_ONE": 32, "KP_MINUS_NEG_Y": 33, "KP_MINUS_SUB_X1": 34, "KP_MINUS_SUB_Y1": 35, "KP_MINUS_G_U1": 36, "KP_MINUS_G_S1": 37, "KP_MINUS_A_2B_X3_SUB": 38,
             "KP_MINUS_A_2B_G_X3_SUB": 39, "ADD_KP_MINUS_SUB_X3": 40, "ADD_KP_MINUS_G_SUB_X3": 41, "ADD": 42, "ADD3": 43, "WORDS": 44, "IS_MULTIPLE_OF_P": 45, "LEAVE": 46,
             "ADD_AFFINE": 64, "ADD_AFFINE_TWIN": 65, "XYZZ_ADD": 66, "XYZZ_LEAVE": 67}
```

Measured after the change: 284,800, median of 4. 1.01x the previous value.
